# awaelchli/torch-optical-flow

Hardware: AMD Instinct MI355X
Metric: image-pairs/sec + corr-lookup HBM GB/s, RAFT 12-iter @ Sintel 1024×436 (higher is better)
Workload: dtype corr + convs split-fp16 (22-bit operands: fp16 hi + lo, 3 f16 MFMA per product, fp32 accumulate); lookup fp32; 1 GPU; raft-12iter-sintel-436x1024; pairs_per_gpu=8, global_batch=8, iters=12, padded=440x1024, parallelism=pairs sharded over 1 GPU(s), conv_benchmark=True, update_impl=split, hip_graph=True, steps_in_flight=1, full=False

## Files before the change

### include/oflow.h

```cpp
#ifndef OFLOW_H_
#define OFLOW_H_

#ifdef __cplusplus
extern "C" {
#endif

#define OFLOW_ABI_VERSION 1

#define OFLOW_OK 0
#define OFLOW_E_NULL (-1)
#define OFLOW_E_SHAPE (-2)
#define OFLOW_E_LEVELS (-3)
#define OFLOW_E_TINY (-4)
#define OFLOW_E_RADIUS (-5)
#define OFLOW_E_MODE (-6)
#define OFLOW_E_ALIGN (-7)

#define OFLOW_MAX_LEVELS 8
#define OFLOW_MAX_RADIUS 7

#define OFLOW_INTERP_BILINEAR 0
#define OFLOW_INTERP_NEAREST 1
#define OFLOW_INTERP_BICUBIC 2
#define OFLOW_PAD_ZEROS 0
#define OFLOW_PAD_BORDER 1
#define OFLOW_PAD_REFLECTION 2

#define OFLOW_IN_S32 0
#define OFLOW_IN_F32_NORM 1
#define OFLOW_IN_F32 2
#define OFLOW_IN_IMG7S2 3
#define OFLOW_IN_FLOW7 4
#define OFLOW_EPI_FLOW_HEAD 3

int oflow_abi_version(void);
const char* oflow_status_string(int status);

int oflow_corr_pyramid_dims(int H, int W, int num_levels, int* level_h, int* level_w);

int oflow_corr_pyramid_f32(const float* d_fmap1, const float* d_fmap2, int B, int C, int H, int W,
                           int num_levels, float* const* d_levels, void* stream);

int oflow_corr_lookup_f32(const float* const* d_levels, const int* level_h, const int* level_w,
                          int num_levels, const float* d_coords, int B, int H, int W, int radius,
                          float* d_out, void* stream);

long long oflow_corr_tiled_level_floats(int H_l, int W_l);
int oflow_corr_pyramid_tiled_f32(const float* d_fmap1, const float* d_fmap2, int B, int C, int H, int W,
                                 int num_levels, float* const* d_levels, void* stream);
int oflow_corr_pyramid_tiled_s32(const void* d_fmap1_s32, const void* d_fmap2_s32, int B, int C, int H, int W,
                                 int num_levels, float* const* d_levels, void* stream);
int oflow_corr_lookup_tiled_f32(const float* const* d_levels, const int* level_h, const int* level_w,
                                int num_levels, const float* d_coords, int B, int H, int W, int radius,
                                float* d_out, void* stream);
int oflow_corr_untile_f32(const float* d_tiled, float* d_out, long long Q, int H_l, int W_l, void* stream);

int oflow_grid_warp_f32(const float* d_frame, const float* d_flow, int B, int C, int H, int W, int mode,
                        int padding_mode, int align_corners, float* d_out, void* stream);

int oflow_grid_sample_f32(const float* d_input, const float* d_grid, int B, int C, int H, int W, int Ho, int Wo,
                          int mode, int padding_mode, int align_corners, float* d_out, void* stream);

int oflow_corr_otf_prepare_f16(const float* d_fmap1, const float* d_fmap2, int B, int C, int H, int W,
                               int num_levels, void* d_f1h, void* const* d_f2h, float* d_scratch, void* stream);
int oflow_corr_lookup_otf_f16(const void* d_f1h, const void* const* d_f2h, const int* level_h, const int* level_w,
                              int num_levels, const float* d_coords, int B, int C, int H, int W, int radius,
                              float* d_out, void* stream);

int oflow_bias_act_f32(const float* d_x, long long sx, const float* d_bias, float* d_y0, long long sy0, float* d_y1,
                       long long sy1, int B, int C, int P, int activation, float scale, void* stream);
int oflow_gru_reset_f32(const float* d_zr, long long szr, const float* d_br, const float* d_h, long long sh,
                        float* d_rh, long long srh, int B, int CH, int P, void* stream);
int oflow_gru_blend_f32(const float* d_zr, long long szr, const float* d_bz, const float* d_q, long long sq,
                        const float* d_bq, float* d_h, long long sh, int B, int CH, int P, void* stream);

int oflow_conv_s32(const void* d_x, long long x_pixel_stride, int in_groups, const void* d_wpack, int n_pad,
                   const float* d_wscale, const float* d_bias, int N, int B, int H, int W, int kh, int kw, int block_n,
                   int epilogue, int activation, float out_scale, void* d_y0, long long y0_pixel_stride, void* d_y1,
                   long long y1_pixel_stride, float* d_f32, long long f32_batch_stride, long long f32_channel_stride,
                   int f32_accumulate, float* d_gru_h, float* d_gru_z, int gru_channels, void* stream);
int oflow_pack_s32_f32(const float* d_x, long long x_batch_stride, int C, int B, int H, int W, int activation,
                       int dst_channel, void* d_y0, long long y0_pixel_stride, void* d_y1, long long y1_pixel_stride,
                       float* d_nhwc, int nhwc_pixel_stride, void* stream);
int oflow_flow_prep_s32(const float* d_coords, int B, int H, int W, void* d_patches, void* d_flow0,
                        long long flow0_pixel_stride, void* d_flow1, long long flow1_pixel_stride, void* stream);
int oflow_flow_head_col2im_f32(const float* d_y, const float* d_bias, int B, int H, int W, float* d_coords, void* stream);
int oflow_flow_head_finish_f32(const float* d_partial, int slabs, const float* d_bias, int B, int H, int W,
                               float* d_coords, void* d_flow0, long long flow0_pixel_stride, void* d_flow1,
                               long long flow1_pixel_stride, void* stream);

int oflow_normalize_images_f32(const float* d_x0, const float* d_x1, long long n, float* d_y0, float* d_y1, void* stream);

int oflow_replicate_pad_f32(const float* const* d_src, float* const* d_dst, int count, long long planes, int H, int W,
                            int top, int bottom, int left, int right, void* stream);

int oflow_set_range_flag(unsigned int* d_flag);

int oflow_range_flag_exchange(unsigned int* d_flag, unsigned int* d_out, void* stream);

int oflow_timing_event_create(void** ev);
int oflow_timing_event_destroy(void* ev);
int oflow_timing_event_record(void* ev, void* stream, int external);
int oflow_timing_event_elapsed_ms(void* start, void* end, float* ms);

int oflow_flow_head2_s32(const void* d_x, long long x_pixel_stride, int in_groups, const float* d_weight,
                         const float* d_bias, int B, int H, int W, float* d_coords, void* stream);
int oflow_flow_head2_tiled_s32(const void* d_x, long long x_pixel_stride, int in_groups, const float* d_wr,
                               const float* d_bias, int B, int H, int W, float* d_coords, void* stream);
int oflow_corr_lookup_tiled_nhwc_f32(const float* const* d_levels, const int* level_h, const int* level_w, int num_levels,
                                     const float* d_coords, int B, int H, int W, int radius, float* d_out, int row_floats,
                                     void* stream);
int oflow_corr_lookup_convc1_s32(const float* const* d_levels, const int* level_h, const int* level_w, int num_levels,
                                 const float* d_coords, int B, int H, int W, int radius, const void* d_wpack,
                                 const float* d_wscale, const float* d_bias, void* d_y, long long y_pixel_stride,
                                 void* stream);

int oflow_conv_s32_ex(const void* d_x, long long x_pixel_stride, int in_groups, const void* d_wpack, int n_pad,
                      const float* d_wscale, const float* d_bias, int N, int B, int H, int W, int kh, int kw,
                      int block_n, int epilogue, int activation, float out_scale, void* d_y0, long long y0_pixel_stride,
                      void* d_y1, long long y1_pixel_stride, float* d_f32, long long f32_batch_stride,
                      long long f32_channel_stride, int f32_accumulate, float* d_gru_h, float* d_gru_z,
                      int gru_channels, float* d_nhwc, int nhwc_pixel_stride, float* d_stats, const void* d_res,
                      long long res_pixel_stride, int res_activation, int s2d, void* stream);
int oflow_conv_s32_ex2(const void* d_x, long long x_pixel_stride, int in_groups, const void* d_wpack, int n_pad,
                       const float* d_wscale, const float* d_bias, int N, int B, int H, int W, int kh, int kw,
                       int block_n, int epilogue, int activation, float out_scale, void* d_y0, long long y0_pixel_stride,
                       void* d_y1, long long y1_pixel_stride, float* d_f32, long long f32_batch_stride,
                       long long f32_channel_stride, int f32_accumulate, float* d_gru_h, float* d_gru_z,
                       int gru_channels, float* d_nhwc, int nhwc_pixel_stride, float* d_stats, const void* d_res,
                       long long res_pixel_stride, int res_activation, int s2d, int in_format,
                       const float* d_in_scale, const float* d_in_shift, void* stream);
int oflow_conv_s32_ex3(const void* d_x, long long x_pixel_stride, int in_groups, const void* d_wpack, int n_pad,
                       const float* d_wscale, const float* d_bias, int N, int B, int H, int W, int kh, int kw,
                       int block_n, int epilogue, int activation, float out_scale, void* d_y0, long long y0_pixel_stride,
                       void* d_y1, long long y1_pixel_stride, float* d_f32, long long f32_batch_stride,
                       long long f32_channel_stride, int f32_accumulate, float* d_gru_h, float* d_gru_z,
                       int gru_channels, float* d_nhwc, int nhwc_pixel_stride, float* d_stats, const void* d_res,
                       long long res_pixel_stride, int res_activation, int s2d, int in_format,
                       const float* d_in_scale, const float* d_in_shift, const float* d_addend,
                       long long addend_pixel_stride, void* stream);
int oflow_conv_s32_ex4(const void* d_x, long long x_pixel_stride, int in_groups, const void* d_wpack, int n_pad,
                       const float* d_wscale, const float* d_bias, int N, int B, int H, int W, int kh, int kw,
                       int block_n, int epilogue, int activation, float out_scale, void* d_y0, long long y0_pixel_stride,
                       void* d_y1, long long y1_pixel_stride, float* d_f32, long long f32_batch_stride,
                       long long f32_channel_stride, int f32_accumulate, float* d_gru_h, float* d_gru_z,
                       int gru_channels, float* d_nhwc, int nhwc_pixel_stride, float* d_stats, const void* d_res,
                       long long res_pixel_stride, int res_activation, int s2d, int in_format,
                       const float* d_in_scale, const float* d_in_shift, const float* d_addend,
                       long long addend_pixel_stride, const void* d_wfrag, void* stream);
int oflow_conv_s32_ex5(const void* d_x, long long x_pixel_stride, int in_groups, const void* d_wpack, int n_pad,
                       const float* d_wscale, const float* d_bias, int N, int B, int H, int W, int kh, int kw,
                       int block_n, int epilogue, int activation, float out_scale, void* d_y0, long long y0_pixel_stride,
                       void* d_y1, long long y1_pixel_stride, float* d_f32, long long f32_batch_stride,
                       long long f32_channel_stride, int f32_accumulate, float* d_gru_h, float* d_gru_z,
                       int gru_channels, float* d_nhwc, int nhwc_pixel_stride, float* d_stats, const void* d_res,
                       long long res_pixel_stride, int res_activation, int s2d, int in_format,
                       const float* d_in_scale, const float* d_in_shift, const float* d_addend,
                       long long addend_pixel_stride, const void* d_wfrag, float* d_ksplit_slab,
                       unsigned* d_ksplit_ctr, long long ksplit_tiles, void* stream);
int oflow_conv_s32_ex6(const void* d_x, long long x_pixel_stride, int in_groups, const void* d_wpack, int n_pad,
                       const float* d_wscale, const float* d_bias, int N, int B, int H, int W, int kh, int kw,
                       int block_n, int epilogue, int activation, float out_scale, void* d_y0, long long y0_pixel_stride,
                       void* d_y1, long long y1_pixel_stride, float* d_f32, long long f32_batch_stride,
                       long long f32_channel_stride, int f32_accumulate, float* d_gru_h, float* d_gru_z,
                       int gru_channels, float* d_nhwc, int nhwc_pixel_stride, float* d_stats, const void* d_res,
                       long long res_pixel_stride, int res_activation, int s2d, int in_format,
                       const float* d_in_scale, const float* d_in_shift, const float* d_addend,
                       long long addend_pixel_stride, const void* d_wfrag, float* d_ksplit_slab,
                       unsigned* d_ksplit_ctr, long long ksplit_tiles, const float* d_fh_weights, float* d_fh_partial,
                       int fh_slabs, void* stream);
int oflow_stem_patches_s32(const float* d_img, int B, int C, int H, int W, void* d_out, int out_groups, void* stream);
int oflow_norm_stats_finalize(const float* d_partials, int B, int tiles, int n_pad, int C, double eps, float* d_alpha,
                              float* d_beta, void* stream);
int oflow_norm_apply_s32(const float* d_x, int C, int B, int H, int W, const float* d_alpha, const float* d_beta,
                         int activation, int res_mode, const void* d_res, long long res_pixel_stride, const float* d_x2,
                         const float* d_alpha2, const float* d_beta2, int res_activation, int s2d, void* d_y,
                         long long y_pixel_stride, void* stream);

int oflow_convex_upsample_f32(const float* d_flow, const float* d_mask, int B, int H, int W, float* d_out, void* stream);

int oflow_corr_lookup_backward_f32(const float* d_grad_out, const float* d_coords, int B, int H, int W, int radius,
                                   float* const* d_grad_levels, const int* level_h, const int* level_w, int num_levels,
                                   void* stream);
int oflow_corr_pyramid_grad_combine_f32(float* const* d_grad_levels, const int* level_h, const int* level_w,
                                        int num_levels, long long Q, void* stream);
int oflow_corr_fmap_grad_f32(const float* d_fmap1, const float* d_fmap2, const float* d_g0, int B, int C, int N,
                             float scale, float* d_grad_f1, float* d_grad_f2, void* stream);

int oflow_grid_warp_backward_f32(const float* d_grad_out, const float* d_frame, const float* d_flow, int B, int C, int H,
                                 int W, int mode, int padding_mode, int align_corners, float* d_grad_frame,
                                 float* d_grad_flow, void* stream);
int oflow_grid_sample_backward_f32(const float* d_grad_out, const float* d_input, const float* d_grid, int B, int C,
                                   int H, int W, int Ho, int Wo, int mode, int padding_mode, int align_corners,
                                   float* d_grad_input, float* d_grad_grid, void* stream);

#define OFLOW_FLOW_STATS_CHUNKS 128
#define OFLOW_FLOW2RGB_BAKER 0
#define OFLOW_FLOW2RGB_HSV 1
#define OFLOW_FLOW2RGB_MEISTER 2
int oflow_flow_stats_f32(const float* d_flow, int B, int H, int W, int clip, float clip_lo, float clip_hi,
                         int invert_y, float* d_partials, void* stream);
int oflow_flow2rgb_f32(const float* d_flow, int B, int H, int W, int method, int clip, float clip_lo, float clip_hi,
                       int invert_y, int have_denom, float denom, const float* d_partials, float* d_rgb, void* stream);
int oflow_flow_pack_f32(const float* d_flow, int B, int H, int W, int channels, int flip_rows, float* d_out,
                        void* stream);

#define OFLOW_FLOW_METRICS_PARTIALS 1024
#define OFLOW_MAX_PREDS 32
#define OFLOW_VALID_NONE 0
#define OFLOW_VALID_F32 1
#define OFLOW_VALID_U8 2
int oflow_flow_error_stats_f32(const float* d_pred, long long pred_sb, long long pred_sc, long long pred_sh,
                               const float* d_target, long long target_sb, long long target_sc, long long target_sh,
                               const void* d_valid, int valid_kind, long long valid_sb, long long valid_sh, int B, int H,
                               int W, float abs_threshold, float rel_threshold, float max_flow, float* d_epe_map,
                               double* d_workspace, double* d_accum, void* stream);
int oflow_sequence_loss_f32(const float* const* d_preds, int n_preds, const float* weights, const float* d_flow_gt,
                            const void* d_valid, int valid_kind, int B, int H, int W, float max_flow,
                            double* d_workspace, float* d_loss, double* d_stats, void* stream);
int oflow_sequence_loss_backward_f32(const float* d_grad_out, const float* const* d_preds, float* const* d_grads,
                                     int n_preds, const float* weights, const float* d_flow_gt, const void* d_valid,
                                     int valid_kind, int B, int H, int W, float max_flow, void* stream);

#ifdef __cplusplus
}
#endif

#endif
```

### torch-optical-flow_amd/csrc/conv_s32.hip

```cpp
#include "oflow_internal.h"

namespace oflow {
namespace {

typedef _Float16 half8 __attribute__((ext_vector_type(8)));
typedef float f32x16 __attribute__((ext_vector_type(16)));
typedef unsigned int u32x4 __attribute__((ext_vector_type(4)));

__device__ __forceinline__ int swz(int row) { return (row >> 1) & 7; }
#ifndef OFLOW_BREG_RING
#define OFLOW_BREG_RING 2
#endif
#ifndef OFLOW_VSLIDE
#define OFLOW_VSLIDE 1
#endif
#ifndef OFLOW_XCD_MAP
#define OFLOW_XCD_MAP 0
#endif
#ifndef OFLOW_STEM_SINGLE_A
#define OFLOW_STEM_SINGLE_A 1
#endif
#ifndef OFLOW_PAD_ROWS
#define OFLOW_PAD_ROWS 1
#endif
#ifndef OFLOW_HALO_DB
#define OFLOW_HALO_DB 0
#endif

constexpr int kTY = 4, kTX = 32;

#ifdef OFLOW_ABLATE
#define OFLOW_ABL(bit) ((a.exp_flags & (bit)) != 0)
#else
#define OFLOW_ABL(bit) false
#endif
constexpr int kAinGroups = 4;


struct ConvArgs {
  const uint8_t* x;
  long long xps;
  int kg;
  const uint8_t* w;
  int npad;
  const float* wsc;
  const float* bias;
  int N;
  int B, H, W, tiles_x, tiles_y;
  int act;
  float oscale;
  uint8_t* y0;
  long long y0ps;
  uint8_t* y1;
  long long y1ps;
  float* f;
  long long fbs, fcs;
  int faccum;
  float* h;
  float* z;
  int gch;
  const float* add;
  long long addps;
  float* fn;
  int fnps;
  float* stats;
  const uint8_t* res;
  long long resps;
  int res_act;
  int s2d;
  const float* ia;
  const float* ib;
  int ain;
  int cin;
  int wbytes;
  const uint8_t* wf;
  int exp_flags;
  float* ks_slab;
  unsigned* ks_ctr;
  long long ks_tiles;
  const float* fhw;
  float* fhy;
};
constexpr int kEpiFlowHead = OFLOW_EPI_FLOW_HEAD;
constexpr int kInS32 = OFLOW_IN_S32, kInF32Norm = OFLOW_IN_F32_NORM, kInF32 = OFLOW_IN_F32, kInImg = OFLOW_IN_IMG7S2,
              kInFlow = OFLOW_IN_FLOW7;
constexpr int kImgC = 3, kImgK = 7, kImgRows = (kTY - 1) * 2 + kImgK, kImgCols = (kTX - 1) * 2 + kImgK;
constexpr int kImgHalf = (kImgCols + 1) / 2, kImgPitch = 2 * kImgHalf, kImgPlane = kImgRows * kImgPitch;

__device__ __forceinline__ float sigmoid_hw(float v) {
  return __builtin_amdgcn_rcpf(1.0f + __builtin_amdgcn_exp2f(v * -1.4426950408889634f));
}
__device__ __forceinline__ float tanh_hw(float v) {
  return 1.0f - 2.0f * __builtin_amdgcn_rcpf(__builtin_amdgcn_exp2f(v * 2.8853900817779268f) + 1.0f);
}

__device__ __forceinline__ float act_fn(float v, int act) {
  if (act == 1) return v < 0.f ? 0.f : v;
  if (act == 2) return 1.0f / (1.0f + expf(-v));
  if (act == 3) return tanhf(v);
  return v;
}

__device__ __forceinline__ void split8(const float* v, half8& hi, half8& lo) { split_vec(v, hi, lo); }

__device__ __forceinline__ void store_s32(uint8_t* y, long long ps, long long P, int n, int N, const float* v, float& gm) {
  uint8_t* line = y + P * ps + (long long)(n >> 5) * 128 + ((n & 31) >> 3) * 16;
  if (n + 8 <= N) {
    half8 hi, lo;
    split8(v, hi, lo);
    gm = fmaxf(gm, fmaxf(fmaxf(fmaxf(fabsf(v[0]), fabsf(v[1])), fmaxf(fabsf(v[2]), fabsf(v[3]))),
                         fmaxf(fmaxf(fabsf(v[4]), fabsf(v[5])), fmaxf(fabsf(v[6]), fabsf(v[7])))));
    *reinterpret_cast<half8*>(line) = hi;
    *reinterpret_cast<half8*>(line + 64) = lo;
  } else {
    _Float16* hp = reinterpret_cast<_Float16*>(line);
    _Float16* lp = reinterpret_cast<_Float16*>(line + 64);
#pragma unroll
    for (int j = 0; j < 8; ++j) {
      if (n + j < N) {
        gm = fmaxf(gm, fabsf(v[j]));
        _Float16 h_, l_;
        split_f16(v[j], h_, l_);
        hp[j] = h_;
        lp[j] = l_;
      }
    }
  }
}

typedef __attribute__((address_space(4))) const float cfloat;
template <int T0, int T1>
__device__ __forceinline__ void flow_head_partials(const float* tp, cfloat* w, float* yp, long long plane, bool in) {
  constexpr int NO = 2 * (T1 - T0);
  float acc[2][NO];
#pragma unroll
  for (int j = 0; j < NO; ++j) acc[0][j] = acc[1][j] = 0.f;
  float wn[2][NO];
#pragma unroll
  for (int e = 0; e < 2; ++e)
#pragma unroll
    for (int j = 0; j < NO; ++j) wn[e][j] = w[e * 18 + 2 * T0 + j];
  float2 tn = *reinterpret_cast<const float2*>(tp);
#pragma unroll
  for (int e = 0; e < 2; ++e)
#pragma unroll
    for (int j = 0; j < NO; ++j) asm volatile("" : "+s"(wn[e][j]));
  asm volatile("" : "+v"(tn.x), "+v"(tn.y));
#pragma unroll 2
  for (int c0 = 0; c0 < 64; c0 += 2) {
    float wc[2][NO];
#pragma unroll
    for (int e = 0; e < 2; ++e)
#pragma unroll
      for (int j = 0; j < NO; ++j) wc[e][j] = wn[e][j];
    const float2 t = tn;
    const int c1 = c0 + 2 < 64 ? c0 + 2 : c0;
#pragma unroll
    for (int e = 0; e < 2; ++e)
#pragma unroll
      for (int j = 0; j < NO; ++j) wn[e][j] = w[(c1 + e) * 18 + 2 * T0 + j];
    tn = *reinterpret_cast<const float2*>(tp + c1);
    __builtin_amdgcn_sched_barrier(0);
#pragma unroll
    for (int j = 0; j < NO; ++j) {
      acc[0][j] = fmaf(t.x, wc[0][j], acc[0][j]);
      acc[1][j] = fmaf(t.y, wc[1][j], acc[1][j]);
    }
    __builtin_amdgcn_sched_barrier(0);
#pragma unroll
    for (int e = 0; e < 2; ++e)
#pragma unroll
      for (int j = 0; j < NO; ++j) asm volatile("" : "+s"(wn[e][j]));
    asm volatile("" : "+v"(tn.x), "+v"(tn.y));
  }
  if (in) {
#pragma unroll
    for (int j = 0; j < NO; ++j) yp[(2 * T0 + j) * plane] = acc[0][j] + acc[1][j];
  }
}

template <int KH, int KW, int BN, int WM, int WN, int EPI, int TY = kTY, int AIN = kInS32, bool BREG = false, int BD = 1>
__global__ __launch_bounds__(64 * WM * WN, WM * WN == 8 ? 1 : 2) void conv_s32_kernel(ConvArgs a) {
  constexpr int NTH = 64 * WM * WN;
  constexpr int T = KH * KW;
  constexpr int BM = TY * kTX;
  constexpr int PH = KH / 2, PW = KW / 2;
  constexpr int HY = TY + KH - 1, HX = kTX + KW - 1, NPIX = HY * HX;
  constexpr int AITEMS = NPIX * 8, APER = (AITEMS + NTH - 1) / NTH;
  constexpr int BITEMS = BN * 8, BPER = (BITEMS + NTH - 1) / NTH;
  constexpr int MT = TY / WM;
  constexpr int NT = BN / WN / 32;
  static_assert((WM * WN == 4 || WM * WN == 8) && MT >= 1 && NT >= 1, "bad wave grid");
  static_assert(NTH % 8 == 0, "an A item's 16-B chunk is tid & 7");
  constexpr bool WIN = AIN == kInImg || AIN == kInFlow;
  constexpr int WC = AIN == kInFlow ? 2 : kImgC, WS = AIN == kInFlow ? 1 : 2;
  constexpr int WROWS = (kTY - 1) * WS + kImgK, WCOLS = (kTX - 1) * WS + kImgK;
  constexpr int WHALF = WS == 2 ? (WCOLS + 1) / 2 : WCOLS, WPITCH = WS == 2 ? 2 * WHALF : WCOLS;
  constexpr int WPLANE = WROWS * WPITCH;
  constexpr int WKPAD = AIN == kInFlow ? 128 : 160;
  constexpr int WAPER = WIN ? BM * 4 / NTH : 1;
  static_assert(!WIN || (BM * 4) % NTH == 0, "window items");
  static_assert(AIN != kInImg || (WHALF == kImgHalf && WPITCH == kImgPitch && WPLANE == kImgPlane), "stem window");
  constexpr bool ADB = (T == 1) && !(WIN && OFLOW_STEM_SINGLE_A);
  constexpr int RS = 128;
  constexpr int RSA = (BREG || OFLOW_PAD_ROWS) ? 144 : RS, RSB = OFLOW_PAD_ROWS ? 144 : RS;
  constexpr int A_BYTES = NPIX * RSA, B_BYTES = BN * RSB;
  static_assert(!BREG || (T > 1 && (WM == 1 || WM == 2 || WM == 4) && BN == 32 * WN && AIN == kInS32),
                "register-direct B: T > 1, WM x WN waves of one 32-channel tile each");
  constexpr bool HDB = BREG && OFLOW_HALO_DB;
  constexpr int MAIN_BYTES = ((ADB || HDB) ? 2 : 1) * A_BYTES + (BREG ? 0 : 2 * B_BYTES);
  constexpr int TS = BN + 4;
  constexpr int EPI_BYTES = BM * TS * 4;
  constexpr int LDS_BYTES = MAIN_BYTES > EPI_BYTES ? MAIN_BYTES : EPI_BYTES;
  constexpr int kImgZero = WC * WPLANE;
  constexpr int IMG_FLOATS = (kImgZero + 1 + 3) & ~3;
  constexpr int AFF_BYTES = AIN == kInF32Norm ? kAinGroups * 32 * 8
                            : WIN ? IMG_FLOATS * 4 + WKPAD * 4
                            : 0;
  static_assert(!WIN || (T == 1 && TY == kTY), "window input: 1x1 geometry over the patch channels, 4-row tiles");
  __shared__ __attribute__((aligned(16))) uint8_t smem[LDS_BYTES + AFF_BYTES];
  __shared__ float2 sSB[BN];
  __shared__ float3 sStat[EPI == 0 ? WM * BN : 1];
  float2* sAff = reinterpret_cast<float2*>(smem + LDS_BYTES);
  float* sImg = reinterpret_cast<float*>(smem + LDS_BYTES);
  int* sKoff = reinterpret_cast<int*>(smem + LDS_BYTES + (WIN ? IMG_FLOATS * 4 : 0));
  uint8_t* sA = smem;
  uint8_t* sB = smem + (ADB ? 2 : 1) * A_BYTES;

  const int tid = threadIdx.x, lane = tid & 63, wave = tid >> 6;
  const int wm = wave / WN, wn = wave % WN;
  const int r = lane & 31, hh = lane >> 5;
  if constexpr (BREG) {
    if (a.ks_slab != nullptr) {
      const int z = blockIdx.z;
      a.x += (long long)z * a.kg * 128;
      a.wf += (long long)z * a.kg * T * a.npad * 128;
    }
  }
  auto aswz = [](int p) { return (BREG || OFLOW_PAD_ROWS) ? 0 : swz(p); };
  auto bswz = [](int n) { return OFLOW_PAD_ROWS ? 0 : swz(n); };

  int tile, cblk;
  if constexpr (OFLOW_XCD_MAP) {
    const int nblk = a.npad / BN, ntiles = a.tiles_x * a.tiles_y * a.B, bid = blockIdx.x;
    const int full = (ntiles >> 3) * 8 * nblk;
    if (bid < full) {
      const int grp = bid / (8 * nblk), rem = bid - grp * 8 * nblk;
      cblk = rem >> 3;
      tile = grp * 8 + (rem & 7);
    } else {
      const int ntail = ntiles & 7, rem = bid - full;
      cblk = rem / ntail;
      tile = (ntiles & ~7) + (rem - cblk * ntail);
    }
  } else {
    tile = blockIdx.x;
    cblk = blockIdx.y;
  }
  const int tx0 = (tile % a.tiles_x) * kTX;
  tile /= a.tiles_x;
  const int ty0 = (tile % a.tiles_y) * TY;
  const int b = tile / a.tiles_y;
  const int n0 = cblk * BN;
  const long long pix0 = (long long)b * a.H * a.W;

  u32x4 ra[APER], rb[BPER];
  const __amdgpu_buffer_rsrc_t rsA = __builtin_amdgcn_make_buffer_rsrc(
      const_cast<uint8_t*>(a.x + pix0 * a.xps), (short)0, (int)((long long)a.H * a.W * a.xps), 0x00020000);
  const __amdgpu_buffer_rsrc_t rsB =
      __builtin_amdgcn_make_buffer_rsrc(const_cast<uint8_t*>(a.w), (short)0, a.wbytes, 0x00020000);
  auto a_off = [&](int s_, int& col) {
    int t_ = tid;
    asm volatile("" : "+v"(t_));
    const int item = (AITEMS % NTH == 0) ? t_ + s_ * NTH : min(t_ + s_ * NTH, AITEMS - 1);
    const int p = item >> 3, c = item & 7;
    const int gy = ty0 - PH + p / HX, gx = tx0 - PW + p % HX;
    const int cy = min(max(gy, 0), a.H - 1), cx = min(max(gx, 0), a.W - 1);
    col = c * 16;
    return (cy * a.W + cx) * (int)a.xps + (AIN == kInF32 ? 0 : c * 16);
  };
  unsigned aok = 0u;
#pragma unroll
  for (int s_ = 0; s_ < APER; ++s_) {
    const int item = (AITEMS % NTH == 0) ? tid + s_ * NTH : min(tid + s_ * NTH, AITEMS - 1);
    const int p = item >> 3;
    const int gy = ty0 - PH + p / HX, gx = tx0 - PW + p % HX;
    const bool ok = static_cast<unsigned>(gy) < static_cast<unsigned>(a.H) && static_cast<unsigned>(gx) < static_cast<unsigned>(a.W);
    aok |= (ok ? 1u : 0u) << s_;
  }
  int boff[BPER];
#pragma unroll
  for (int s_ = 0; s_ < BPER; ++s_) boff[s_] = (n0 + (tid + s_ * NTH) / 8) * 128 + ((tid + s_ * NTH) & 7) * 16;
#define OFLOW_LOAD_A(RA, G)                                                                                          \
  if constexpr (!WIN) _Pragma("unroll") for (int s_ = 0; s_ < APER; ++s_) {                                        \
    int col_;                                                                                                        \
    const int off_ = a_off(s_, col_);                                                                                \
    if constexpr (AIN == kInF32)    \
      RA[s_] = __builtin_amdgcn_raw_buffer_load_b128(rsA, off_ + min((G) * 128 + col_, a.cin * 4 - 16), 0, 0);      \
    else                                                                                                             \
      RA[s_] = __builtin_amdgcn_raw_buffer_load_b128(rsA, off_, (G) * 128, 0);                                      \
  }
#define OFLOW_WRITE_A(RA, BUF, G)                                                                                    \
  if (!OFLOW_ABL(4)) {                                                                                               \
  float amx_ = 0.f;                                                                                                  \
  float2 af4_[4];                                                                                                    \
  if constexpr (AIN == kInF32Norm) _Pragma("unroll") for (int e_ = 0; e_ < 4; ++e_)                                  \
    af4_[e_] = sAff[(G) * 32 + 4 * (tid & 7) + e_];                                                                  \
  if constexpr (WIN) {                                                                                               \
                                                                                                        \
    _Pragma("unroll") for (int s_ = 0; s_ < WAPER; ++s_) {                                                           \
      const int item = tid + s_ * NTH;                                                                               \
      const int p = item % BM, cp = item / BM;                                                                       \
      const int pb_ = WS * (p >> 5) * WPITCH + (p & 31);                                                             \
      const int4 k0_ = *reinterpret_cast<const int4*>(sKoff + (G) * 32 + 8 * cp);                                    \
      const int4 k1_ = *reinterpret_cast<const int4*>(sKoff + (G) * 32 + 8 * cp + 4);                                \
      const int kov_[8] = {k0_.x, k0_.y, k0_.z, k0_.w, k1_.x, k1_.y, k1_.z, k1_.w};                                  \
      float v8_[8];                                                                                                  \
      _Pragma("unroll") for (int e_ = 0; e_ < 8; ++e_) {                                                             \
        v8_[e_] = sImg[kov_[e_] < 0 ? kImgZero : pb_ + kov_[e_]];                                                    \
        amx_ = fmaxf(amx_, fabsf(v8_[e_]));                                                                          \
      }                                                                                                              \
      half8 h8_, l8_;                                                                                                \
      split_vec(v8_, h8_, l8_);                                                                                      \
      uint8_t* rw_ = sA + (BUF) * A_BYTES + p * RSA;                                                                 \
      *reinterpret_cast<half8*>(rw_ + ((cp ^ aswz(p)) << 4)) = h8_;                                                  \
      *reinterpret_cast<half8*>(rw_ + (((4 + cp) ^ aswz(p)) << 4)) = l8_;                                            \
    }                                                                                                                \
  } else                                                                                                             \
  _Pragma("unroll") for (int s_ = 0; s_ < APER; ++s_) {                                                              \
    const int item = tid + s_ * NTH;                                                                            \
                                                     \
    const int p = item >> 3, c = item & 7;                                                                           \
    if (AITEMS % NTH == 0 || item < AITEMS) {                                                                   \
      if constexpr (AIN != kInS32) {                                                                                 \
                   \
        typedef _Float16 half4_ __attribute__((ext_vector_type(4)));                                                 \
        half4_ h4 = {0, 0, 0, 0}, l4 = {0, 0, 0, 0};                                                                 \
        if (((aok >> s_) & 1u) && (AIN != kInF32 || (G) * 32 + 4 * c < a.cin)) {                                     \
          const float* fv = reinterpret_cast<const float*>(&RA[s_]);                                                 \
          float mx_ = 0.f, v4_[4];                                                                                   \
          _Pragma("unroll") for (int e_ = 0; e_ < 4; ++e_) {                                                         \
            float v_ = fv[e_];                                                                                       \
            if constexpr (AIN == kInF32Norm) {                                                                       \
              const float2 af = af4_[e_];                                                                            \
              v_ = v_ * af.x + af.y;                                                                                 \
              v_ = v_ < 0.f ? 0.f : v_;                                                                              \
            }                                                                                                        \
            mx_ = fmaxf(mx_, fabsf(v_));                                                                             \
            v4_[e_] = v_;                                                                                            \
          }                                                                                                          \
          split_vec(v4_, h4, l4);                                                                                    \
          amx_ = fmaxf(amx_, mx_);                                                                                   \
        }                                                                                                            \
        uint8_t* rw_ = sA + (BUF) * A_BYTES + p * RSA + (c & 1) * 8;                                                 \
        *reinterpret_cast<half4_*>(rw_ + (((c >> 1) ^ aswz(p)) << 4)) = h4;                                          \
        *reinterpret_cast<half4_*>(rw_ + (((4 + (c >> 1)) ^ aswz(p)) << 4)) = l4;                                    \
      } else {                                                                                                       \
        *reinterpret_cast<u32x4*>(sA + (BUF) * A_BYTES + p * RSA + ((c ^ aswz(p)) << 4)) =                          \
            ((aok >> s_) & 1u) ? RA[s_] : u32x4{0u, 0u, 0u, 0u};                                                     \
      }                                                                                                              \
    }                                                                                                                \
  }                                                                                                                  \
  if constexpr (AIN != kInS32) range_guard(amx_);                                                                    \
  }
#define OFLOW_LOAD_B(RB, STEP)                                                                                       \
  _Pragma("unroll") for (int s_ = 0; s_ < BPER; ++s_) {                                                              \
    const int item = tid + s_ * NTH;                                                                            \
    if (BITEMS % NTH == 0 || item < BITEMS)                                                                     \
      RB[s_] = __builtin_amdgcn_raw_buffer_load_b128(rsB, boff[s_], (STEP) * a.npad * 128, 0);                      \
  }
#define OFLOW_WRITE_B(RB, BUF)                                                                                       \
  if (!OFLOW_ABL(32)) _Pragma("unroll") for (int s_ = 0; s_ < BPER; ++s_) {                                          \
    const int item = tid + s_ * NTH;                                                                            \
    const int n = item >> 3, c = item & 7;                                                                           \
    if (BITEMS % NTH == 0 || item < BITEMS)                                                                     \
      *reinterpret_cast<u32x4*>(sB + (BUF) * B_BYTES + n * RSB + ((c ^ bswz(n)) << 4)) = RB[s_];                    \
  }
#define OFLOW_READ_OPS(AH, AL, BH, BL, I, S_)                                                                        \
  {                                                                                                                  \
    const int ii_ = (I);                                                                                              \
    const int t_ = ii_ % T, ky_ = t_ / KW, kx_ = t_ - ky_ * KW;                                                       \
    const uint8_t* bufA_ = sA + (ADB ? (ii_ & 1) * A_BYTES : 0);                                                      \
    const uint8_t* bufB_ = sB + (ii_ & 1) * B_BYTES;                                                                  \
    const int chi_ = 2 * (S_) + hh, clo_ = 4 + 2 * (S_) + hh;                                                        \
    _Pragma("unroll") for (int mt_ = 0; mt_ < MT; ++mt_) {                                                           \
      const int p_ = (wm * MT + mt_ + ky_) * HX + r + kx_;                                                           \
      const uint8_t* row_ = bufA_ + p_ * RSA;                                                                        \
      AH[mt_] = *reinterpret_cast<const half8*>(row_ + ((chi_ ^ aswz(p_)) << 4));                                    \
      AL[mt_] = *reinterpret_cast<const half8*>(row_ + ((clo_ ^ aswz(p_)) << 4));                                    \
    }                                                                                                                \
    _Pragma("unroll") for (int nt_ = 0; nt_ < NT; ++nt_) {                                                           \
      const int n_ = wn * (BN / WN) + nt_ * 32 + r;                                                                  \
      const uint8_t* row_ = bufB_ + n_ * RSB;                                                                        \
      BH[nt_] = *reinterpret_cast<const half8*>(row_ + ((chi_ ^ bswz(n_)) << 4));                                    \
      BL[nt_] = *reinterpret_cast<const half8*>(row_ + ((clo_ ^ bswz(n_)) << 4));                                    \
    }                                                                                                                \
  }
#define OFLOW_MFMAS(AH, AL, BH, BL)                                                                                  \
  if (!OFLOW_ABL(2)) _Pragma("unroll") for (int mt = 0; mt < MT; ++mt)                                               \
    _Pragma("unroll") for (int nt = 0; nt < NT; ++nt) {                                                              \
      acc[mt][nt] = __builtin_amdgcn_mfma_f32_32x32x16_f16(AH[mt], BL[nt], acc[mt][nt], 0, 0, 0);                    \
      acc[mt][nt] = __builtin_amdgcn_mfma_f32_32x32x16_f16(AL[mt], BH[nt], acc[mt][nt], 0, 0, 0);                    \
      acc[mt][nt] = __builtin_amdgcn_mfma_f32_32x32x16_f16(AH[mt], BH[nt], acc[mt][nt], 0, 0, 0);                    \
    }

  f32x16 acc[MT][NT];
#pragma unroll
  for (int i = 0; i < MT; ++i)
#pragma unroll
    for (int j = 0; j < NT; ++j)
#pragma unroll
      for (int e = 0; e < 16; ++e) acc[i][j][e] = 0.f;

  const int S = a.kg * T;
  for (int c = tid; c < BN; c += NTH) {
    const int n = min(n0 + c, a.N - 1);
    sSB[c] = make_float2(a.wsc[n], a.bias ? a.bias[n] : 0.f);
  }
  if constexpr (AIN == kInF32Norm) {
    for (int e = tid; e < a.kg * 32; e += NTH)
      sAff[e] = make_float2(a.ia[(long long)b * a.kg * 32 + e], a.ib[(long long)b * a.kg * 32 + e]);
    __syncthreads();
  }
  if constexpr (AIN == kInImg) {
    const float* img = reinterpret_cast<const float*>(a.x) + (long long)b * kImgC * (2 * a.H) * (2 * a.W);
    const int iy0 = 2 * ty0 - kImgK / 2, ix0 = 2 * tx0 - kImgK / 2;
    constexpr int IMG_N = kImgC * kImgRows * kImgCols, IMG_PER = (IMG_N + NTH - 1) / NTH;
    if (a.exp_flags & 1) {
      for (int e = tid; e < IMG_N; e += NTH) {
        const int ch = e / (kImgRows * kImgCols), rem = e - ch * (kImgRows * kImgCols);
        const int ry = rem / kImgCols, rx = rem - ry * kImgCols;
        const int iy = iy0 + ry, ix = ix0 + rx;
        float v = 0.f;
        if (static_cast<unsigned>(iy) < static_cast<unsigned>(2 * a.H) && static_cast<unsigned>(ix) < static_cast<unsigned>(2 * a.W))
          v = img[((long long)ch * (2 * a.H) + iy) * (2 * a.W) + ix];
        sImg[ch * kImgPlane + ry * kImgPitch + (rx & 1) * kImgHalf + (rx >> 1)] = v;
      }
    } else {
    float iv[IMG_PER];
    int io[IMG_PER];
#pragma unroll
    for (int s_ = 0; s_ < IMG_PER; ++s_) {
      const int e = min(tid + s_ * NTH, IMG_N - 1);
      const int ch = e / (kImgRows * kImgCols), rem = e - ch * (kImgRows * kImgCols);
      const int ry = rem / kImgCols, rx = rem - ry * kImgCols;
      const int iy = iy0 + ry, ix = ix0 + rx;
      const bool in = static_cast<unsigned>(iy) < static_cast<unsigned>(2 * a.H) && static_cast<unsigned>(ix) < static_cast<unsigned>(2 * a.W);
      const int cy = min(max(iy, 0), 2 * a.H - 1), cx = min(max(ix, 0), 2 * a.W - 1);
      const float v = img[((long long)ch * (2 * a.H) + cy) * (2 * a.W) + cx];
      iv[s_] = in ? v : 0.f;
      io[s_] = ch * kImgPlane + ry * kImgPitch + (rx & 1) * kImgHalf + (rx >> 1);
    }
#pragma unroll
    for (int s_ = 0; s_ < IMG_PER; ++s_)
      if (tid + s_ * NTH < IMG_N) sImg[io[s_]] = iv[s_];
    }
  }
  if constexpr (AIN == kInFlow) {
    const float* co = reinterpret_cast<const float*>(a.x) + (long long)b * 2 * a.H * a.W;
    const int iy0 = ty0 - kImgK / 2, ix0 = tx0 - kImgK / 2;
    constexpr int FL_N = 2 * WROWS * WCOLS, FL_PER = (FL_N + NTH - 1) / NTH;
    float iv[FL_PER];
    int io[FL_PER];
#pragma unroll
    for (int s_ = 0; s_ < FL_PER; ++s_) {
      const int e = min(tid + s_ * NTH, FL_N - 1);
      const int ch = e / (WROWS * WCOLS), rem = e - ch * (WROWS * WCOLS);
      const int ry = rem / WCOLS, rx = rem - ry * WCOLS;
      const int iy = iy0 + ry, ix = ix0 + rx;
      const bool in = static_cast<unsigned>(iy) < static_cast<unsigned>(a.H) && static_cast<unsigned>(ix) < static_cast<unsigned>(a.W);
      const int cy = min(max(iy, 0), a.H - 1), cx = min(max(ix, 0), a.W - 1);
      const float v = co[((long long)ch * a.H + cy) * a.W + cx] - static_cast<float>(ch == 0 ? ix : iy);
      iv[s_] = in ? v : 0.f;
      io[s_] = ch * WPLANE + ry * WPITCH + rx;
    }
#pragma unroll
    for (int s_ = 0; s_ < FL_PER; ++s_)
      if (tid + s_ * NTH < FL_N) sImg[io[s_]] = iv[s_];
  }
  if constexpr (WIN) {
    for (int k = tid; k < WKPAD; k += NTH) {
      const int t = k / WC, ch = k - t * WC;
      const int ky = t / kImgK, kx = t - ky * kImgK;
      sKoff[k] = t < kImgK * kImgK
                     ? ch * WPLANE + ky * WPITCH + (WS == 2 ? (kx & 1) * WHALF + (kx >> 1) : kx)
                     : -1;
    }
    if (tid == 0) sImg[kImgZero] = 0.f;
    __syncthreads();
  }
  if constexpr (BREG) {
  const __amdgpu_buffer_rsrc_t rsW =
      __builtin_amdgcn_make_buffer_rsrc(const_cast<uint8_t*>(a.wf), (short)0, a.wbytes, 0x00020000);
  const int wlane = ((n0 >> 5) + wn) * 4096 + lane * 16;
  const int wstep = a.npad * 128;
  constexpr int RING = (T == 5 && KH == 5 && EPI == 0) ? 2 : OFLOW_BREG_RING;
  u32x4 bq[RING][4];
  auto load_b = [&](u32x4 (&d)[4], int step) {
#pragma unroll
    for (int e = 0; e < 4; ++e) d[e] = __builtin_amdgcn_raw_buffer_load_b128(rsW, wlane + e * 1024, step * wstep, 0);
  };
#define OFLOW_READ_A(AH, AL, I, S_)                                                                                   \
  {                                                                                                                  \
    const int ii_ = (I);                                                                                              \
    const int t_ = ii_ % T, ky_ = t_ / KW, kx_ = t_ - ky_ * KW;                                                       \
    const int chi_ = 2 * (S_) + hh, clo_ = 4 + 2 * (S_) + hh;                                                        \
    const uint8_t* sAb_ = sA + (HDB && ((ii_ / T) & 1) ? A_BYTES : 0);           \
    _Pragma("unroll") for (int mt_ = 0; mt_ < MT; ++mt_) {                                                           \
      const int p_ = (wm * MT + mt_ + ky_) * HX + r + kx_;                                                           \
      const uint8_t* row_ = sAb_ + p_ * RSA;                                                                         \
      AH[mt_] = *reinterpret_cast<const half8*>(row_ + (chi_ << 4));                                                 \
      AL[mt_] = *reinterpret_cast<const half8*>(row_ + (clo_ << 4));                                                 \
    }                                                                                                                \
  }
#define OFLOW_MFMAS_R(AH, AL, BC, S_)                                                                                 \
  if (!OFLOW_ABL(2)) _Pragma("unroll") for (int mt = 0; mt < MT; ++mt) {                                             \
    const half8 bh_ = __builtin_bit_cast(half8, BC[2 * (S_)]), bl_ = __builtin_bit_cast(half8, BC[2 * (S_) + 1]);     \
    acc[mt][0] = __builtin_amdgcn_mfma_f32_32x32x16_f16(AH[mt], bl_, acc[mt][0], 0, 0, 0);                           \
    acc[mt][0] = __builtin_amdgcn_mfma_f32_32x32x16_f16(AL[mt], bh_, acc[mt][0], 0, 0, 0);                           \
    acc[mt][0] = __builtin_amdgcn_mfma_f32_32x32x16_f16(AH[mt], bh_, acc[mt][0], 0, 0, 0);                           \
  }
#pragma unroll
  for (int q = 0; q < RING; ++q) load_b(bq[q], q < S ? q : S - 1);
  OFLOW_LOAD_A(ra, 0);
  OFLOW_WRITE_A(ra, 0, 0);
  OFLOW_LOAD_A(ra, a.kg > 1 ? 1 : 0);
  __syncthreads();
  constexpr int GPB = (T % RING == 0) ? 1 : RING;
  constexpr bool VSLIDE = OFLOW_VSLIDE && KW == 1 && KH > 1 && WM == 1 && !(EPI == 0 && KH == 5);
  if constexpr (VSLIDE) {
    constexpr int NR = MT + KH - 1;
    half8 V[NR][2][2];
    auto rd = [&](int hr, int sub, int grp) {
      const uint8_t* row_ = sA + (HDB && (grp & 1) ? A_BYTES : 0) + (hr * HX + r) * RSA;
      V[hr][sub][0] = *reinterpret_cast<const half8*>(row_ + ((2 * sub + hh) << 4));
      V[hr][sub][1] = *reinterpret_cast<const half8*>(row_ + ((4 + 2 * sub + hh) << 4));
    };
    auto mf = [&](int ky, int sub, u32x4 (&bc)[4]) {
      if (OFLOW_ABL(2)) return;
      const half8 bh_ = __builtin_bit_cast(half8, bc[2 * sub]), bl_ = __builtin_bit_cast(half8, bc[2 * sub + 1]);
#pragma unroll
      for (int mt = 0; mt < MT; ++mt) {
        acc[mt][0] = __builtin_amdgcn_mfma_f32_32x32x16_f16(V[mt + ky][sub][0], bl_, acc[mt][0], 0, 0, 0);
        acc[mt][0] = __builtin_amdgcn_mfma_f32_32x32x16_f16(V[mt + ky][sub][1], bh_, acc[mt][0], 0, 0, 0);
        acc[mt][0] = __builtin_amdgcn_mfma_f32_32x32x16_f16(V[mt + ky][sub][0], bh_, acc[mt][0], 0, 0, 0);
      }
    };
#pragma unroll
    for (int m = 0; m < MT; ++m) rd(m, 0, 0);
    for (int g0 = 0; g0 < a.kg; g0 += GPB) {
#pragma unroll
      for (int j = 0; j < GPB * T; ++j) {
        const int gg = g0 + j / T, t = j % T;
        if (GPB > 1 && j > 0 && t == 0 && gg >= a.kg) break;
        const int i_ = gg * T + t;
        u32x4 (&bc)[4] = bq[j % RING];
        if (t == 0) {
#pragma unroll
          for (int m = 0; m < MT; ++m) rd(m, 1, gg);
        } else {
          rd(t + MT - 1, 1, gg);
        }
        mf(t, 0, bc);
        if (t == T - 1) {
          if constexpr (HDB) {
            OFLOW_WRITE_A(ra, (gg + 1) & 1, gg + 1 < a.kg ? gg + 1 : gg);
          } else {
            __syncthreads();
            OFLOW_WRITE_A(ra, 0, gg + 1 < a.kg ? gg + 1 : gg);
          }
          const int g2 = gg + 2 < a.kg ? gg + 2 : a.kg - 1;
          OFLOW_LOAD_A(ra, g2);
          __syncthreads();
#pragma unroll
          for (int m = 0; m < MT; ++m) rd(m, 0, gg + 1);
        } else {
          rd(t + MT, 0, gg);
        }
        mf(t, 1, bc);
        load_b(bc, i_ + RING < S ? i_ + RING : S - 1);
      }
    }
  } else {
  half8 xah[MT], xal[MT], yah[MT], yal[MT];
  OFLOW_READ_A(xah, xal, 0, 0);
  for (int g0 = 0; g0 < a.kg; g0 += GPB) {
#pragma unroll
    for (int j = 0; j < GPB * T; ++j) {
      const int gg = g0 + j / T, t = j % T;
      if (GPB > 1 && j > 0 && t == 0 && gg >= a.kg) break;
      const int i_ = gg * T + t;
      u32x4 (&bc)[4] = bq[j % RING];
      OFLOW_READ_A(yah, yal, i_, 1);
      OFLOW_MFMAS_R(xah, xal, bc, 0);
      if (t == T - 1) {
        if constexpr (HDB) {
          OFLOW_WRITE_A(ra, (gg + 1) & 1, gg + 1 < a.kg ? gg + 1 : gg);
        } else {
          __syncthreads();
          OFLOW_WRITE_A(ra, 0, gg + 1 < a.kg ? gg + 1 : gg);
        }
        const int g2 = gg + 2 < a.kg ? gg + 2 : a.kg - 1;
        OFLOW_LOAD_A(ra, g2);
        __syncthreads();
      }
      OFLOW_READ_A(xah, xal, i_ + 1, 0);
      OFLOW_MFMAS_R(yah, yal, bc, 1);
      load_b(bc, i_ + RING < S ? i_ + RING : S - 1);
    }
  }
  }
#undef OFLOW_READ_A
#undef OFLOW_MFMAS_R
  } else {
  u32x4 rbr[BD][BPER];
  u32x4 rar[ADB ? BD : 1][APER];
  OFLOW_LOAD_B(rbr[0], 0);
  OFLOW_LOAD_A(rar[0], 0);
  OFLOW_WRITE_A(rar[0], 0, 0);
  OFLOW_WRITE_B(rbr[0], 0);
#pragma unroll
  for (int d = 1; d <= BD; ++d) {
    const int id = d < S ? d : S - 1;
    OFLOW_LOAD_B(rbr[d % BD], id);
    if constexpr (ADB) { OFLOW_LOAD_A(rar[d % BD], id); }
  }
  if constexpr (!ADB) { OFLOW_LOAD_A(rar[0], a.kg > 1 ? 1 : 0); }
  __syncthreads();
  half8 xah[MT], xal[MT], xbh[NT], xbl[NT];
  half8 yah[MT], yal[MT], ybh[NT], ybl[NT];
  OFLOW_READ_OPS(xah, xal, xbh, xbl, 0, 0);

  constexpr int GPB2 = (BD > 1 && (T % BD) != 0) ? BD : 1;
  for (int g0 = 0; g0 < a.kg; g0 += GPB2) {
#pragma unroll
    for (int j = 0; j < GPB2 * T; ++j) {
      const int g = g0 + j / T, t = j % T;
      if (GPB2 > 1 && j > 0 && t == 0 && g >= a.kg) break;
      const int i_ = g * T + t;
      u32x4 (&rb)[BPER] = rbr[(j + 1) % BD];
      OFLOW_WRITE_B(rb, (i_ + 1) & 1);
      if constexpr (ADB) { OFLOW_WRITE_A(rar[(j + 1) % BD], (i_ + 1) & 1, i_ + 1 < S ? i_ + 1 : S - 1); }
      {
        const int i2 = i_ + 1 + BD < S ? i_ + 1 + BD : S - 1;
        OFLOW_LOAD_B(rb, i2);
        if constexpr (ADB) { OFLOW_LOAD_A(rar[(j + 1) % BD], i2); }
      }
      OFLOW_READ_OPS(yah, yal, ybh, ybl, i_, 1);
      OFLOW_MFMAS(xah, xal, xbh, xbl);
      if constexpr (!ADB) {
        if (t == T - 1) {
          __syncthreads();
          OFLOW_WRITE_A(rar[0], 0, g + 1 < a.kg ? g + 1 : g);
          const int g2 = g + 2 < a.kg ? g + 2 : a.kg - 1;
          OFLOW_LOAD_A(rar[0], g2);
        }
      }
      if (!OFLOW_ABL(64)) __syncthreads();
      OFLOW_READ_OPS(xah, xal, xbh, xbl, i_ + 1, 0);
      OFLOW_MFMAS(yah, yal, ybh, ybl);
    }
  }
  }
#undef OFLOW_MFMAS
#undef OFLOW_READ_OPS
#undef OFLOW_LOAD_A
#undef OFLOW_WRITE_A
#undef OFLOW_LOAD_B
#undef OFLOW_WRITE_B

  if constexpr (BREG) {
    if (a.ks_slab != nullptr) {
      typedef __attribute__((address_space(1))) unsigned gu32;
      __shared__ unsigned sTicket;
      const int tile_id = blockIdx.y * gridDim.x + blockIdx.x;
      gu32* ctr = (gu32*)(a.ks_ctr) + 2 * tile_id;
      if (tid == 0) sTicket = __hip_atomic_fetch_add(ctr, 1u, __ATOMIC_RELAXED, __HIP_MEMORY_SCOPE_AGENT);
      __syncthreads();
      const unsigned ticket = sTicket;
      const __amdgpu_buffer_rsrc_t rsS = __builtin_amdgcn_make_buffer_rsrc(
          a.ks_slab + (size_t)tile_id * (BM * BN), (short)0, BM * BN * 4, 0x00020000);
      const int sbase = wave * (MT * NT * 4096) + lane * 16;
      if ((ticket & 1u) == 0u) {
#pragma unroll
        for (int mt = 0; mt < MT; ++mt)
#pragma unroll
          for (int nt = 0; nt < NT; ++nt)
#pragma unroll
            for (int e4 = 0; e4 < 4; ++e4) {
              const u32x4 v = {__float_as_uint(acc[mt][nt][4 * e4]), __float_as_uint(acc[mt][nt][4 * e4 + 1]),
                               __float_as_uint(acc[mt][nt][4 * e4 + 2]), __float_as_uint(acc[mt][nt][4 * e4 + 3])};
              __builtin_amdgcn_raw_buffer_store_b128(v, rsS, sbase + ((mt * NT + nt) * 4 + e4) * 1024, 0, 16);
            }
        asm volatile("s_waitcnt vmcnt(0)" ::: "memory");
        __syncthreads();
        if (tid == 0) __hip_atomic_fetch_add(ctr + 1, 1u, __ATOMIC_RELAXED, __HIP_MEMORY_SCOPE_AGENT);
        return;
      }
      if (tid == 0) {
        const unsigned want = (ticket >> 1) + 1u;
        for (unsigned spin = 0; spin < (1u << 24); ++spin) {
          if (static_cast<int>(__hip_atomic_load(ctr + 1, __ATOMIC_RELAXED, __HIP_MEMORY_SCOPE_AGENT) - want) >= 0) break;
          __builtin_amdgcn_s_sleep(1);
        }
        __builtin_amdgcn_fence(__ATOMIC_ACQUIRE, "agent");
        asm volatile("s_waitcnt vmcnt(0)" ::: "memory");
      }
      __syncthreads();
#pragma unroll
      for (int mt = 0; mt < MT; ++mt)
#pragma unroll
        for (int nt = 0; nt < NT; ++nt) {
          u32x4 pv[4];
#pragma unroll
          for (int e4 = 0; e4 < 4; ++e4)
            pv[e4] = __builtin_amdgcn_raw_buffer_load_b128(rsS, sbase + ((mt * NT + nt) * 4 + e4) * 1024, 0, 0);
#pragma unroll
          for (int e4 = 0; e4 < 4; ++e4)
#pragma unroll
            for (int j = 0; j < 4; ++j) acc[mt][nt][4 * e4 + j] += __uint_as_float(pv[e4][j]);
        }
    }
  }

  constexpr int C8 = BN / 8;
  constexpr int KIT = (BM * C8 + NTH - 1) / NTH;
  constexpr bool GRU = EPI == 1 || EPI == 2;
  const bool has_add = GRU && a.add != nullptr;
  u32x4 ad[GRU ? KIT : 1][2];
  if (has_add) {
#pragma unroll
    for (int k = 0; k < (GRU ? KIT : 0); ++k) {
      const int item = tid + k * NTH;
      const int pl = item / C8, n = n0 + (item - pl * C8) * 8;
      const int y = ty0 + pl / kTX, x = tx0 + (pl % kTX);
      if (item >= BM * C8 || n >= a.N || y >= a.H || x >= a.W) continue;
      const u32x4* ap = reinterpret_cast<const u32x4*>(a.add + (pix0 + (long long)y * a.W + x) * a.addps + n);
      ad[k][0] = ap[0];
      ad[k][1] = ap[1];
    }
  }
  __syncthreads();
  float* sT = reinterpret_cast<float*>(smem);
#pragma unroll
  for (int mt = 0; mt < MT; ++mt)
#pragma unroll
    for (int nt = 0; nt < NT; ++nt) {
      const int nl = wn * (BN / WN) + nt * 32 + r;
      const int pbase = (wm * MT + mt) * kTX;
      if constexpr (EPI == kEpiFlowHead) {
        const float2 sb = sSB[nl];
#pragma unroll
        for (int e = 0; e < 16; ++e) {
          const int m = (e & 3) + 8 * (e >> 2) + 4 * hh;
          const float v = fmaf(acc[mt][nt][e], sb.x, sb.y);
          sT[(pbase + m) * TS + nl] = v < 0.f ? 0.f : v;
        }
      } else {
#pragma unroll
      for (int e = 0; e < 16; ++e) {
        const int m = (e & 3) + 8 * (e >> 2) + 4 * hh;
        sT[(pbase + m) * TS + nl] = acc[mt][nt][e];
      }
      }
    }
  if constexpr (EPI == 0 && TY >= kTY) {
    if (a.stats != nullptr && !OFLOW_ABL(8)) {
#pragma unroll
      for (int nt = 0; nt < NT; ++nt) {
        const int nl = wn * (BN / WN) + nt * 32 + r;
        const float2 sb = sSB[nl];
        float cnt = 0.f, sum = 0.f, q = 0.f;
        const bool full = ty0 + TY <= a.H && tx0 + kTX <= a.W;
        if (full) {
#pragma unroll
          for (int mt = 0; mt < MT; ++mt)
#pragma unroll
            for (int e = 0; e < 16; ++e) sum += acc[mt][nt][e] * sb.x + sb.y;
          cnt = 16.f * MT;
        } else {
#pragma unroll
          for (int mt = 0; mt < MT; ++mt) {
            const bool yok = ty0 + wm * MT + mt < a.H;
#pragma unroll
            for (int e = 0; e < 16; ++e) {
              const bool ok = yok && tx0 + (e & 3) + 8 * (e >> 2) + 4 * hh < a.W;
              sum += ok ? acc[mt][nt][e] * sb.x + sb.y : 0.f;
              cnt += ok ? 1.f : 0.f;
            }
          }
        }
        const float mean = cnt > 0.f ? sum / cnt : 0.f;
        if (full) {
#pragma unroll
          for (int mt = 0; mt < MT; ++mt)
#pragma unroll
            for (int e = 0; e < 16; ++e) {
              const float d = (acc[mt][nt][e] * sb.x + sb.y) - mean;
              float dd = d * d;
              asm volatile("" : "+v"(dd));
              q += dd;
            }
        } else {
#pragma unroll
          for (int mt = 0; mt < MT; ++mt) {
            const bool yok = ty0 + wm * MT + mt < a.H;
#pragma unroll
            for (int e = 0; e < 16; ++e) {
              const bool ok = yok && tx0 + (e & 3) + 8 * (e >> 2) + 4 * hh < a.W;
              const float d = (acc[mt][nt][e] * sb.x + sb.y) - mean;
              q += ok ? d * d : 0.f;
            }
          }
        }
        const float nb = __shfl_xor(cnt, 32), mb = __shfl_xor(mean, 32), qb = __shfl_xor(q, 32);
        const float n0_ = hh ? nb : cnt, m0_ = hh ? mb : mean, q0_ = hh ? qb : q;
        const float n1_ = hh ? cnt : nb, m1_ = hh ? mean : mb, q1_ = hh ? q : qb;
        const float nn = n0_ + n1_;
// ... 445 lines not shown

using namespace oflow;

extern "C" int oflow_conv_s32_ex5(const void* d_x, long long x_pixel_stride, int in_groups, const void* d_wpack,
                                  int n_pad, const float* d_wscale, const float* d_bias, int N, int B, int H, int W, int kh,
                                  int kw, int block_n, int epilogue, int activation, float out_scale, void* d_y0,
                                  long long y0_pixel_stride, void* d_y1, long long y1_pixel_stride, float* d_f32,
                                  long long f32_batch_stride, long long f32_channel_stride, int f32_accumulate,
                                  float* d_gru_h, float* d_gru_z, int gru_channels, float* d_nhwc, int nhwc_pixel_stride,
                                  float* d_stats, const void* d_res, long long res_pixel_stride, int res_activation,
                                  int s2d, int in_format, const float* d_in_scale, const float* d_in_shift,
                                  const float* d_addend, long long addend_pixel_stride, const void* d_wfrag,
                                  float* d_ksplit_slab, unsigned* d_ksplit_ctr, long long ksplit_tiles, void* stream);

extern "C" int oflow_conv_s32_ex4(const void* d_x, long long x_pixel_stride, int in_groups, const void* d_wpack,
                                  int n_pad, const float* d_wscale, const float* d_bias, int N, int B, int H, int W, int kh,
                                  int kw, int block_n, int epilogue, int activation, float out_scale, void* d_y0,
                                  long long y0_pixel_stride, void* d_y1, long long y1_pixel_stride, float* d_f32,
                                  long long f32_batch_stride, long long f32_channel_stride, int f32_accumulate,
                                  float* d_gru_h, float* d_gru_z, int gru_channels, float* d_nhwc, int nhwc_pixel_stride,
                                  float* d_stats, const void* d_res, long long res_pixel_stride, int res_activation,
                                  int s2d, int in_format, const float* d_in_scale, const float* d_in_shift,
                                  const float* d_addend, long long addend_pixel_stride, const void* d_wfrag, void* stream) {
  return oflow_conv_s32_ex5(d_x, x_pixel_stride, in_groups, d_wpack, n_pad, d_wscale, d_bias, N, B, H, W, kh, kw,
                            block_n, epilogue, activation, out_scale, d_y0, y0_pixel_stride, d_y1, y1_pixel_stride,
                            d_f32, f32_batch_stride, f32_channel_stride, f32_accumulate, d_gru_h, d_gru_z, gru_channels,
                            d_nhwc, nhwc_pixel_stride, d_stats, d_res, res_pixel_stride, res_activation, s2d, in_format,
                            d_in_scale, d_in_shift, d_addend, addend_pixel_stride, d_wfrag, nullptr, nullptr, 0, stream);
}

extern "C" int oflow_conv_s32_ex5(const void* d_x, long long x_pixel_stride, int in_groups, const void* d_wpack,
                                  int n_pad, const float* d_wscale, const float* d_bias, int N, int B, int H, int W, int kh,
                                  int kw, int block_n, int epilogue, int activation, float out_scale, void* d_y0,
                                  long long y0_pixel_stride, void* d_y1, long long y1_pixel_stride, float* d_f32,
                                  long long f32_batch_stride, long long f32_channel_stride, int f32_accumulate,
                                  float* d_gru_h, float* d_gru_z, int gru_channels, float* d_nhwc, int nhwc_pixel_stride,
                                  float* d_stats, const void* d_res, long long res_pixel_stride, int res_activation,
                                  int s2d, int in_format, const float* d_in_scale, const float* d_in_shift,
                                  const float* d_addend, long long addend_pixel_stride, const void* d_wfrag,
                                  float* d_ksplit_slab, unsigned* d_ksplit_ctr, long long ksplit_tiles, void* stream) {
  ConvArgs a;
  const int st = build_conv_args(a, d_x, x_pixel_stride, in_groups, d_wpack, n_pad, d_wscale, d_bias, N, B, H, W, kh, kw,
                                 block_n, epilogue, activation, out_scale, d_y0, y0_pixel_stride, d_y1, y1_pixel_stride,
                                 d_f32, f32_batch_stride, f32_channel_stride, f32_accumulate, d_gru_h, d_gru_z,
                                 gru_channels, d_nhwc, nhwc_pixel_stride, d_stats, d_res, res_pixel_stride,
                                 res_activation, s2d);
  if (st != OFLOW_OK) return st;
  if (d_wfrag) {
    if ((uintptr_t)d_wfrag & 15) return OFLOW_E_ALIGN;
    if (n_pad % 32) return OFLOW_E_SHAPE;
    a.wf = static_cast<const uint8_t*>(d_wfrag);
  }
  if (in_format < kInS32 || in_format > kInFlow) return OFLOW_E_MODE;
  if (in_format == kInFlow) {
    if (kh != 1 || kw != 1 || epilogue != 0 || block_n != 128 || in_groups != (kImgK * kImgK * 2 + 31) / 32)
      return OFLOW_E_MODE;
    if ((long long)2 * B * H * W >= (1ll << 31) || d_addend) return OFLOW_E_SHAPE;
    a.ain = in_format;
    return dispatch_conv(a, kh, kw, block_n, epilogue, static_cast<hipStream_t>(stream));
  }
  if (in_format == kInImg) {
    if (kh != 1 || kw != 1 || epilogue != 0 || block_n != 64 || in_groups != (kImgK * kImgK * kImgC + 31) / 32)
      return OFLOW_E_MODE;
    if ((long long)kImgC * 4 * H * W >= (1ll << 31)) return OFLOW_E_SHAPE;
    a.ain = in_format;
    if (d_addend) return OFLOW_E_MODE;
    return dispatch_conv(a, kh, kw, block_n, epilogue, static_cast<hipStream_t>(stream));
  }
  if (in_format != kInF32 && (x_pixel_stride & 127)) return OFLOW_E_ALIGN;
  if (in_format == kInF32Norm && x_pixel_stride != (long long)in_groups * 128) return OFLOW_E_SHAPE;
  if (in_format == kInF32) {
    const long long cin = x_pixel_stride / 4;
    if ((x_pixel_stride & 15) || cin > (long long)in_groups * 32 || cin <= (long long)(in_groups - 1) * 32) return OFLOW_E_SHAPE;
    a.cin = static_cast<int>(cin);
  }
  if (in_format == kInF32Norm) {
    if (!d_in_scale || !d_in_shift) return OFLOW_E_NULL;
    if (kh != 3 || kw != 3 || epilogue != 0 || in_groups > kAinGroups) return OFLOW_E_MODE;
    a.ia = d_in_scale;
    a.ib = d_in_shift;
  } else if (in_format == kInF32) {
    if (kh != 1 || kw != 1 || epilogue != 0 || block_n != 128) return OFLOW_E_MODE;
  }
  a.ain = in_format;
  if (d_addend) {
    if (epilogue == 0) return OFLOW_E_MODE;
    if (N % 8) return OFLOW_E_SHAPE;
    if (((uintptr_t)d_addend & 15) || (addend_pixel_stride & 3) || addend_pixel_stride < N) return OFLOW_E_ALIGN;
    a.add = d_addend;
    a.addps = addend_pixel_stride;
  }
  if (d_ksplit_slab || d_ksplit_ctr) {
    if (!d_ksplit_slab || !d_ksplit_ctr) return OFLOW_E_NULL;
    if (((uintptr_t)d_ksplit_slab & 15) || ((uintptr_t)d_ksplit_ctr & 7)) return OFLOW_E_ALIGN;
    if (ksplit_tiles <= 0) return OFLOW_E_SHAPE;
    a.ks_slab = d_ksplit_slab;
    const bool breg = in_format == kInS32 && a.wf != nullptr && use_breg(a, block_n, kh * kw) && kh * kw != 4 &&
                      (block_n == 128 || (kh == 3 && kw == 3)) && (epilogue == 0 || kh * kw == 5);
    a.ks_slab = nullptr;
    if (breg && (in_groups % 2) == 0) {
      if ((long long)B * ((H + kTY - 1) / kTY) * ((W + kTX - 1) / kTX) * (n_pad / block_n) > ksplit_tiles)
        return OFLOW_E_SHAPE;
      a.ks_slab = d_ksplit_slab;
      a.ks_ctr = d_ksplit_ctr;
      a.ks_tiles = ksplit_tiles;
      a.kg = in_groups / 2;
      a.wbytes /= 2;
    }
  }
  return dispatch_conv(a, kh, kw, block_n, epilogue, static_cast<hipStream_t>(stream));
}

extern "C" int oflow_conv_s32_ex6(const void* d_x, long long x_pixel_stride, int in_groups, const void* d_wpack,
                                  int n_pad, const float* d_wscale, const float* d_bias, int N, int B, int H, int W, int kh,
                                  int kw, int block_n, int epilogue, int activation, float out_scale, void* d_y0,
                                  long long y0_pixel_stride, void* d_y1, long long y1_pixel_stride, float* d_f32,
                                  long long f32_batch_stride, long long f32_channel_stride, int f32_accumulate,
                                  float* d_gru_h, float* d_gru_z, int gru_channels, float* d_nhwc, int nhwc_pixel_stride,
                                  float* d_stats, const void* d_res, long long res_pixel_stride, int res_activation,
                                  int s2d, int in_format, const float* d_in_scale, const float* d_in_shift,
                                  const float* d_addend, long long addend_pixel_stride, const void* d_wfrag,
                                  float* d_ksplit_slab, unsigned* d_ksplit_ctr, long long ksplit_tiles,
                                  const float* d_fh_weights, float* d_fh_partial, int fh_slabs, void* stream) {
  if (epilogue != kEpiFlowHead)
    return oflow_conv_s32_ex5(d_x, x_pixel_stride, in_groups, d_wpack, n_pad, d_wscale, d_bias, N, B, H, W, kh, kw,
                              block_n, epilogue, activation, out_scale, d_y0, y0_pixel_stride, d_y1, y1_pixel_stride,
                              d_f32, f32_batch_stride, f32_channel_stride, f32_accumulate, d_gru_h, d_gru_z,
                              gru_channels, d_nhwc, nhwc_pixel_stride, d_stats, d_res, res_pixel_stride, res_activation,
                              s2d, in_format, d_in_scale, d_in_shift, d_addend, addend_pixel_stride, d_wfrag,
                              d_ksplit_slab, d_ksplit_ctr, ksplit_tiles, stream);
  if (!d_fh_weights || !d_fh_partial) return OFLOW_E_NULL;
  if (N != 256 || n_pad != 256 || fh_slabs != N / 64 || kh != 3 || kw != 3 || (block_n != 64 && block_n != 128))
    return OFLOW_E_SHAPE;
  if (in_format != kInS32 || activation != 1 || out_scale != 1.0f || d_y0 || d_y1 || d_f32 || d_gru_h || d_gru_z ||
      d_nhwc || d_stats || d_res || s2d || d_addend || d_ksplit_slab || d_ksplit_ctr)
    return OFLOW_E_MODE;
  if ((x_pixel_stride & 127) || ((uintptr_t)d_fh_weights & 3) || ((uintptr_t)d_fh_partial & 3)) return OFLOW_E_ALIGN;
  ConvArgs a;
  const int st = build_conv_args(a, d_x, x_pixel_stride, in_groups, d_wpack, n_pad, d_wscale, d_bias, N, B, H, W, kh, kw,
                                 block_n, 0, activation, out_scale, nullptr, 0, nullptr, 0, d_fh_partial, 0, 0, 0, nullptr,
                                 nullptr, 0, nullptr, 0, nullptr, nullptr, 0, 0, 0);
  if (st != OFLOW_OK) return st;
  a.f = nullptr;
  a.fhw = d_fh_weights;
  a.fhy = d_fh_partial;
  if (d_wfrag) {
    if ((uintptr_t)d_wfrag & 15) return OFLOW_E_ALIGN;
    a.wf = static_cast<const uint8_t*>(d_wfrag);
  }
  a.ain = kInS32;
  return dispatch_conv(a, kh, kw, block_n, epilogue, static_cast<hipStream_t>(stream));
}

extern "C" int oflow_conv_s32_ex3(const void* d_x, long long x_pixel_stride, int in_groups, const void* d_wpack,
                                  int n_pad, const float* d_wscale, const float* d_bias, int N, int B, int H, int W, int kh,
                                  int kw, int block_n, int epilogue, int activation, float out_scale, void* d_y0,
                                  long long y0_pixel_stride, void* d_y1, long long y1_pixel_stride, float* d_f32,
                                  long long f32_batch_stride, long long f32_channel_stride, int f32_accumulate,
                                  float* d_gru_h, float* d_gru_z, int gru_channels, float* d_nhwc, int nhwc_pixel_stride,
                                  float* d_stats, const void* d_res, long long res_pixel_stride, int res_activation,
                                  int s2d, int in_format, const float* d_in_scale, const float* d_in_shift,
                                  const float* d_addend, long long addend_pixel_stride, void* stream) {
  return oflow_conv_s32_ex4(d_x, x_pixel_stride, in_groups, d_wpack, n_pad, d_wscale, d_bias, N, B, H, W, kh, kw,
                            block_n, epilogue, activation, out_scale, d_y0, y0_pixel_stride, d_y1, y1_pixel_stride,
                            d_f32, f32_batch_stride, f32_channel_stride, f32_accumulate, d_gru_h, d_gru_z, gru_channels,
                            d_nhwc, nhwc_pixel_stride, d_stats, d_res, res_pixel_stride, res_activation, s2d, in_format,
                            d_in_scale, d_in_shift, d_addend, addend_pixel_stride, nullptr, stream);
}

extern "C" int oflow_conv_s32_ex2(const void* d_x, long long x_pixel_stride, int in_groups, const void* d_wpack,
                                  int n_pad, const float* d_wscale, const float* d_bias, int N, int B, int H, int W, int kh,
                                  int kw, int block_n, int epilogue, int activation, float out_scale, void* d_y0,
                                  long long y0_pixel_stride, void* d_y1, long long y1_pixel_stride, float* d_f32,
                                  long long f32_batch_stride, long long f32_channel_stride, int f32_accumulate,
                                  float* d_gru_h, float* d_gru_z, int gru_channels, float* d_nhwc, int nhwc_pixel_stride,
                                  float* d_stats, const void* d_res, long long res_pixel_stride, int res_activation,
                                  int s2d, int in_format, const float* d_in_scale, const float* d_in_shift,
                                  void* stream) {
  return oflow_conv_s32_ex3(d_x, x_pixel_stride, in_groups, d_wpack, n_pad, d_wscale, d_bias, N, B, H, W, kh, kw,
                            block_n, epilogue, activation, out_scale, d_y0, y0_pixel_stride, d_y1, y1_pixel_stride,
                            d_f32, f32_batch_stride, f32_channel_stride, f32_accumulate, d_gru_h, d_gru_z, gru_channels,
                            d_nhwc, nhwc_pixel_stride, d_stats, d_res, res_pixel_stride, res_activation, s2d, in_format,
                            d_in_scale, d_in_shift, nullptr, 0, stream);
}

extern "C" int oflow_conv_s32_ex(const void* d_x, long long x_pixel_stride, int in_groups, const void* d_wpack,
                                 int n_pad, const float* d_wscale, const float* d_bias, int N, int B, int H, int W, int kh,
                                 int kw, int block_n, int epilogue, int activation, float out_scale, void* d_y0,
                                 long long y0_pixel_stride, void* d_y1, long long y1_pixel_stride, float* d_f32,
                                 long long f32_batch_stride, long long f32_channel_stride, int f32_accumulate,
                                 float* d_gru_h, float* d_gru_z, int gru_channels, float* d_nhwc, int nhwc_pixel_stride,
                                 float* d_stats, const void* d_res, long long res_pixel_stride, int res_activation,
                                 int s2d, void* stream) {
  return oflow_conv_s32_ex2(d_x, x_pixel_stride, in_groups, d_wpack, n_pad, d_wscale, d_bias, N, B, H, W, kh, kw,
                            block_n, epilogue, activation, out_scale, d_y0, y0_pixel_stride, d_y1, y1_pixel_stride,
                            d_f32, f32_batch_stride, f32_channel_stride, f32_accumulate, d_gru_h, d_gru_z, gru_channels,
                            d_nhwc, nhwc_pixel_stride, d_stats, d_res, res_pixel_stride, res_activation, s2d, kInS32,
                            nullptr, nullptr, stream);
}

extern "C" int oflow_conv_s32(const void* d_x, long long x_pixel_stride, int in_groups, const void* d_wpack, int n_pad,
                              const float* d_wscale, const float* d_bias, int N, int B, int H, int W, int kh, int kw,
                              int block_n, int epilogue, int activation, float out_scale, void* d_y0,
                              long long y0_pixel_stride, void* d_y1, long long y1_pixel_stride, float* d_f32,
                              long long f32_batch_stride, long long f32_channel_stride, int f32_accumulate,
                              float* d_gru_h, float* d_gru_z, int gru_channels, void* stream) {
  return oflow_conv_s32_ex(d_x, x_pixel_stride, in_groups, d_wpack, n_pad, d_wscale, d_bias, N, B, H, W, kh, kw,
                           block_n, epilogue, activation, out_scale, d_y0, y0_pixel_stride, d_y1, y1_pixel_stride,
                           d_f32, f32_batch_stride, f32_channel_stride, f32_accumulate, d_gru_h, d_gru_z, gru_channels,
                           nullptr, 0, nullptr, nullptr, 0, 0, 0, stream);
}

extern "C" void oflow_exp_set_small_grid_px(int pixels) { oflow::g_small_grid_px = pixels; }
extern "C" void oflow_exp_set_stats_8row(int on) { oflow::g_stats_8row = on; }
extern "C" void oflow_exp_set_conv_flags(int flags) { oflow::g_conv_exp_flags = flags; }
extern "C" void oflow_exp_set_bn64_8row(int on) { oflow::g_bn64_8row = on; }
```

### torch-optical-flow_amd/methods/raft/model/extractor.py

```python
from __future__ import annotations

import os

from typing import Optional, List, Sequence, Tuple, Union

import torch
import torch.nn as nn
from torch import Tensor

from optical_flow import _native

from .update import CONV_BLOCKS, parse_block_overrides


def _norm_layer(norm_fn: str, planes: int, groups: int) -> nn.Module:
    if norm_fn == "group":
        return nn.GroupNorm(num_groups=groups, num_channels=planes)
    if norm_fn == "batch":
        return nn.BatchNorm2d(planes)
    if norm_fn == "instance":
        return nn.InstanceNorm2d(planes)
    if norm_fn == "none":
        return nn.Sequential()
    raise ValueError(f"unknown norm_fn {norm_fn!r}")


class ResidualBlock(nn.Module):

    def __init__(self, in_planes: int, planes: int, norm_fn: str = "group", stride: int = 1) -> None:
        super().__init__()
        self.conv1 = nn.Conv2d(in_planes, planes, kernel_size=3, padding=1, stride=stride)
        self.conv2 = nn.Conv2d(planes, planes, kernel_size=3, padding=1)
        self.relu = nn.ReLU(inplace=True)
        groups = planes // 8
        self.norm1 = _norm_layer(norm_fn, planes, groups)
        self.norm2 = _norm_layer(norm_fn, planes, groups)
        if stride != 1:
            self.norm3 = _norm_layer(norm_fn, planes, groups)
            self.downsample = nn.Sequential(nn.Conv2d(in_planes, planes, kernel_size=1, stride=stride), self.norm3)
        else:
            self.downsample = None

    def forward(self, x: Tensor) -> Tensor:
        y = self.relu(self.norm1(self.conv1(x)))
        y = self.relu(self.norm2(self.conv2(y)))
        if self.downsample is not None:
            x = self.downsample(x)
        return self.relu(x + y)


class BasicEncoder(nn.Module):

    def __init__(self, output_dim: int = 128, norm_fn: str = "batch", dropout: float = 0.0) -> None:
        super().__init__()
        self.norm_fn = norm_fn
        self.norm1 = _norm_layer(norm_fn, 64, 8)
        self.conv1 = nn.Conv2d(3, 64, kernel_size=7, stride=2, padding=3)
        self.relu1 = nn.ReLU(inplace=True)
        self.in_planes = 64
        self.layer1 = self._make_layer(64, stride=1)
        self.layer2 = self._make_layer(96, stride=2)
        self.layer3 = self._make_layer(128, stride=2)
        self.conv2 = nn.Conv2d(128, output_dim, kernel_size=1)
        self.dropout = nn.Dropout2d(p=dropout) if dropout > 0 else None
        for m in self.modules():
            if isinstance(m, nn.Conv2d):
                nn.init.kaiming_normal_(m.weight, mode="fan_out", nonlinearity="relu")
            elif isinstance(m, (nn.BatchNorm2d, nn.InstanceNorm2d, nn.GroupNorm)):
                if m.weight is not None:
                    nn.init.constant_(m.weight, 1)
                if m.bias is not None:
                    nn.init.constant_(m.bias, 0)

    def _make_layer(self, dim: int, stride: int = 1) -> nn.Module:
        blocks = (ResidualBlock(self.in_planes, dim, self.norm_fn, stride=stride), ResidualBlock(dim, dim, self.norm_fn, 1))
        self.in_planes = dim
        return nn.Sequential(*blocks)

    def forward(self, x: Union[Tensor, Sequence[Tensor]]) -> Union[Tensor, Tuple[Tensor, ...]]:
        is_list = isinstance(x, (tuple, list))
        if is_list:
            batch_dim = x[0].shape[0]
            x = torch.cat(list(x), dim=0)
        x = self.relu1(self.norm1(self.conv1(x)))
        x = self.layer3(self.layer2(self.layer1(x)))
        x = self.conv2(x)
        if self.training and self.dropout is not None:
            x = self.dropout(x)
        if is_list:
            return torch.split(x, [batch_dim, batch_dim], dim=0)
        return x




def _s2d_weight(w: Tensor) -> Tensor:
    n, c = w.shape[:2]
    out = torch.zeros((n, 4, c, 2, 2), device=w.device, dtype=w.dtype)
    for kyp in range(2):
        for a in range(2):
            ky = 2 * kyp + a - 1
            if not 0 <= ky <= 2:
                continue
            for kxp in range(2):
                for b in range(2):
                    kx = 2 * kxp + b - 1
                    if 0 <= kx <= 2:
                        out[:, a * 2 + b, :, kyp, kxp] = w[:, :, ky, kx]
    return out.reshape(n, 4 * c, 2, 2)


def _fold_bn(conv: nn.Conv2d, bn: nn.Module):
    w = conv.weight.detach().double()
    b = conv.bias.detach().double() if conv.bias is not None else torch.zeros(w.shape[0], device=w.device, dtype=w.dtype)
    alpha = bn.weight.detach().double() / torch.sqrt(bn.running_var.detach().double() + bn.eps)
    beta = bn.bias.detach().double() - bn.running_mean.detach().double() * alpha
    return (w * alpha.view(-1, 1, 1, 1)).float(), (b * alpha + beta).float()


_ENC_BN_OVERRIDE = {int(k): v for k, v in
                    parse_block_overrides("OFLOW_ENC_BN", {str(b) for b in CONV_BLOCKS}).items()}


class SplitEncoder:

    def __init__(self, enc: BasicEncoder) -> None:
        if enc.norm_fn not in ("instance", "batch"):
            raise RuntimeError(f"SplitEncoder: norm_fn {enc.norm_fn!r} not supported")
        if enc.norm_fn == "batch" and enc.training:
            raise RuntimeError("SplitEncoder: batch norm needs eval mode (running statistics)")
        self.enc = enc
        self.inorm = enc.norm_fn == "instance"
        from .update import cached_pack, tensor_key

        key = tuple(tensor_key(q) for q in enc.parameters()) + tuple(tensor_key(q) for q in enc.buffers())
        self.w = cached_pack(enc, key, lambda: self._pack(enc))

    def _cw(self, conv: nn.Conv2d, norm, **kw):
        if self.inorm or norm is None:
            w, b = conv.weight, conv.bias
        else:
            w, b = _fold_bn(conv, norm)
        if kw.pop("s2d", False):
            w = _s2d_weight(w.detach().float())
        n = w.shape[0]
        return _native.ConvWeights(w, b, ((n + 31) // 32) * 32, **kw)

    def _pack(self, enc: BasicEncoder):
        W = {"stem": self._cw(enc.conv1, enc.norm1, patches=True)}
        for li, layer in enumerate((enc.layer1, enc.layer2, enc.layer3)):
            for bi, blk in enumerate(layer):
                s2 = blk.downsample is not None
                W[f"{li}.{bi}.conv1"] = self._cw(blk.conv1, blk.norm1, s2d=s2)
                W[f"{li}.{bi}.conv2"] = self._cw(blk.conv2, blk.norm2)
                if s2:
                    W[f"{li}.{bi}.down"] = self._cw(blk.downsample[0], blk.downsample[1])
        W["head"] = _native.ConvWeights(enc.conv2.weight, enc.conv2.bias, ((enc.conv2.out_channels + 31) // 32) * 32)
        return W

    @staticmethod
    def _bn(n: int) -> int:
        bn = {64: 64, 96: 96, 128: 128}.get(n, 128 if n % 128 == 0 else 64 if n % 64 == 0 else 32)
        return _ENC_BN_OVERRIDE.get(bn, bn)

    def _conv_norm(self, x, cw, shape, act, out=None, res=None, s2d=False, raw_only=False):
        b, h, w = shape
        bn = self._bn(cw.n)
        V = _native.S32Slice
        dev = x.device
        if self.inorm:
            raw = torch.empty((b * h * w, cw.n), device=dev, dtype=torch.float32)
            tiles = _native.conv_tiles(h, w)
            part = torch.empty((b, tiles, cw.n_pad, 3), device=dev, dtype=torch.float32)
            _native.conv_s32(x, cw, bn, nhwc=raw, stats=part)
            alpha, beta = _native.norm_stats(part, b, tiles, cw.n_pad, cw.n, 1e-5)
            if raw_only:
                return raw, alpha, beta
            if out is None:
                out = _native.s32_empty(b, h // 2 if s2d else h, w // 2 if s2d else w, (cw.n * (4 if s2d else 1) + 31) // 32, dev)
            if isinstance(res, _native.NhwcNormIn):
                _native.norm_apply(raw, (b, cw.n, h, w), alpha, beta, act, V(out), res_raw=(res.raw, res.scale, res.shift),
                                   res_act="relu", s2d=s2d, res_raw_relu=True)
            elif isinstance(res, tuple):
                _native.norm_apply(raw, (b, cw.n, h, w), alpha, beta, act, V(out), res_raw=res, res_act="relu", s2d=s2d)
            else:
                _native.norm_apply(raw, (b, cw.n, h, w), alpha, beta, act, V(out), res=res, res_act="relu" if res is not None else "none", s2d=s2d)
            return out
        if raw_only:
            out = _native.s32_empty(b, h, w, (cw.n + 31) // 32, dev)
            _native.conv_s32(x, cw, bn, y0=V(out))
            return out
        if out is None:
            out = _native.s32_empty(b, h // 2 if s2d else h, w // 2 if s2d else w, (cw.n * (4 if s2d else 1) + 31) // 32, dev)
        _native.conv_s32(x, cw, bn, act=act, y0=V(out), res=res, res_act="relu" if res is not None else "none", s2d=s2d)
        return out

    def _conv1(self, x, cw, shape):
        if self.inorm:
            raw, alpha, beta = self._conv_norm(x, cw, shape, "relu", raw_only=True)
            return _native.NhwcNormIn(raw, *shape, alpha, beta)
        return _native.S32Slice(self._conv_norm(x, cw, shape, "relu"))

    def stem_patches(self, x: Tensor) -> Tensor:
        x = x.float().contiguous()
        n, _, hh, ww = x.shape
        patches = _native.s32_empty(n, hh // 2, ww // 2, self.w["stem"].kg, x.device)
        _native.stem_patches(x, patches)
        return patches

    def __call__(self, x: Union[Tensor, Sequence[Tensor]], patches: Optional[Tensor] = None,
                 split_out: bool = False, stem_from_image: bool = False) -> Union[Tensor, Tuple[Tensor, ...]]:
        is_list = isinstance(x, (tuple, list))
        if is_list:
            batch_dim = x[0].shape[0]
            n, _, hh, ww = x[0].shape
            n *= len(x)
            if patches is None or tuple(patches.shape[:4]) != (n, hh // 2, ww // 2, self.w["stem"].kg):
                x = torch.cat(list(x), dim=0)
        if not isinstance(x, (tuple, list)):
            x = x.float().contiguous()
            n, _, hh, ww = x.shape
            dev = x.device
        else:
            dev = x[0].device
        if hh % 8 or ww % 8:
            raise RuntimeError("SplitEncoder: H and W must be multiples of 8")
        V = _native.S32Slice
        h, w = hh // 2, ww // 2
        if stem_from_image:
            if isinstance(x, (tuple, list)):
                x = torch.cat([t.float() for t in x], dim=0)
            stem_in = _native.ImgIn(x.float().contiguous())
            self.patches = None
        else:
            if patches is None or tuple(patches.shape[:4]) != (n, h, w, self.w["stem"].kg):
                patches = _native.s32_empty(n, h, w, self.w["stem"].kg, dev)
                _native.stem_patches(x, patches)
            self.patches = patches
            stem_in = V(patches)
        cur = (self._conv1(stem_in, self.w["stem"], (n, h, w)) if self.inorm
               else self._conv_norm(stem_in, self.w["stem"], (n, h, w), "relu"))
        layers = (self.enc.layer1, self.enc.layer2, self.enc.layer3)
        for li, layer in enumerate(layers):
            for bi, blk in enumerate(layer):
                last_of_stage = bi == len(layer) - 1
                out_s2d = last_of_stage and li + 1 < len(layers)
                pre = f"{li}.{bi}."
                if blk.downsample is None:
                    x_in = cur if isinstance(cur, _native.NhwcNormIn) else V(cur)
                    t = self._conv1(x_in, self.w[pre + "conv1"], (n, h, w))
                    cur = self._conv_norm(t, self.w[pre + "conv2"], (n, h, w), "relu", res=x_in, s2d=out_s2d)
                else:
                    h, w = h // 2, w // 2
                    t = self._conv1(V(cur), self.w[pre + "conv1"], (n, h, w))
                    cin = self.w[pre + "down"].kg
                    d = self._conv_norm(V(cur, 0, cin), self.w[pre + "down"], (n, h, w), "none", raw_only=True)
                    res = d if self.inorm else V(d)
                    cur = self._conv_norm(t, self.w[pre + "conv2"], (n, h, w), "relu", res=res, s2d=out_s2d)
                if out_s2d:
                    pass
        head = self.w["head"]
        if split_out:
            out = _native.s32_empty(n, h, w, (head.n + 31) // 32, dev)
            _native.conv_s32(V(cur), head, self._bn(head.n), y0=V(out))
        else:
            out = torch.empty((n, head.n, h, w), device=dev, dtype=torch.float32)
            _native.conv_s32(V(cur), head, self._bn(head.n), f32=out)
        if is_list:
            return torch.split(out, [batch_dim, batch_dim], dim=0)
        return out
```

### torch-optical-flow_amd/methods/raft/model/update.py

```python
from __future__ import annotations

import contextlib
import os
import threading
from typing import Optional, Tuple

import torch
import torch.nn as nn
import torch.nn.functional as F
from torch import Tensor

from optical_flow import _native



CONV_BN = {"c2": 96, "f1": 128, "f2": 64, "mo": 128, "gru": 128, "fh1": 64}
CONV_BN_SIDE = dict(CONV_BN, c2=64, fh1=128)
CONV_BLOCKS = (32, 64, 96, 128)


def parse_block_overrides(var: str, keys) -> dict:
    spec = os.environ.get(var, "")
    out = {}
    for kv in filter(None, (s.strip() for s in spec.split(","))):
        k, sep, v = kv.partition("=")
        if not sep or not v.strip().isdigit():
            raise ValueError(f"{var}={spec!r}: expected comma-separated key=block entries, got {kv!r}")
        key = k.strip()
        if keys is not None and key not in keys:
            raise ValueError(f"{var}={spec!r}: unknown key {key!r} (one of {sorted(keys)})")
        if int(v) not in CONV_BLOCKS:
            raise ValueError(f"{var}={spec!r}: block {v} for {key!r} is not one of {CONV_BLOCKS}")
        out[key] = int(v)
    return out


def _env_choice(var: str, default: str, choices) -> str:
    v = os.environ.get(var, default)
    if v not in choices:
        raise ValueError(f"{var}={v!r}: expected one of {list(choices)}")
    return v


for _bn in (CONV_BN, CONV_BN_SIDE):
    _bn.update(parse_block_overrides("OFLOW_CONV_BN", set(CONV_BN)))
FLOW_HEAD_MODE = _env_choice("OFLOW_FLOW_HEAD_MODE", "fused", ("fused", "tiled", "conv", "col2im"))
CONVF1_FROM_FLOW_MIN_PIXELS = 16384 if _env_choice("OFLOW_CONVF1_FROM_FLOW", "1", ("0", "1")) == "1" else 1 << 62
KSPLIT_LAYERS = frozenset()
KSPLIT_MIN_PIXELS = 16384

class FlowHead(nn.Module):
    def __init__(self, input_dim: int = 128, hidden_dim: int = 256) -> None:
        super().__init__()
        self.conv1 = nn.Conv2d(input_dim, hidden_dim, 3, padding=1)
        self.conv2 = nn.Conv2d(hidden_dim, 2, 3, padding=1)
        self.relu = nn.ReLU(inplace=True)

    def forward(self, x: Tensor) -> Tensor:
        return self.conv2(self.relu(self.conv1(x)))


class SepConvGRU(nn.Module):

    def __init__(self, hidden_dim: int = 128, input_dim: int = 192 + 128) -> None:
        super().__init__()
        cin = hidden_dim + input_dim
        self.convz1 = nn.Conv2d(cin, hidden_dim, (1, 5), padding=(0, 2))
        self.convr1 = nn.Conv2d(cin, hidden_dim, (1, 5), padding=(0, 2))
        self.convq1 = nn.Conv2d(cin, hidden_dim, (1, 5), padding=(0, 2))
        self.convz2 = nn.Conv2d(cin, hidden_dim, (5, 1), padding=(2, 0))
        self.convr2 = nn.Conv2d(cin, hidden_dim, (5, 1), padding=(2, 0))
        self.convq2 = nn.Conv2d(cin, hidden_dim, (5, 1), padding=(2, 0))

    @staticmethod
    def _step(h: Tensor, x: Tensor, convz: nn.Module, convr: nn.Module, convq: nn.Module) -> Tensor:
        hx = torch.cat([h, x], dim=1)
        z = torch.sigmoid(convz(hx))
        r = torch.sigmoid(convr(hx))
        q = torch.tanh(convq(torch.cat([r * h, x], dim=1)))
        return (1 - z) * h + z * q

    def forward(self, h: Tensor, x: Tensor) -> Tensor:
        h = self._step(h, x, self.convz1, self.convr1, self.convq1)
        return self._step(h, x, self.convz2, self.convr2, self.convq2)


class BasicMotionEncoder(nn.Module):

    def __init__(self, corr_levels: int, corr_radius: int) -> None:
        super().__init__()
        corr_planes = corr_levels * (2 * corr_radius + 1) ** 2
        self.convc1 = nn.Conv2d(corr_planes, 256, 1, padding=0)
        self.convc2 = nn.Conv2d(256, 192, 3, padding=1)
        self.convf1 = nn.Conv2d(2, 128, 7, padding=3)
        self.convf2 = nn.Conv2d(128, 64, 3, padding=1)
        self.conv = nn.Conv2d(64 + 192, 128 - 2, 3, padding=1)

    def forward(self, flow: Tensor, corr: Tensor) -> Tensor:
        cor = F.relu(self.convc2(F.relu(self.convc1(corr))))
        flo = F.relu(self.convf2(F.relu(self.convf1(flow))))
        out = F.relu(self.conv(torch.cat([cor, flo], dim=1)))
        return torch.cat([out, flow], dim=1)


class BasicUpdateBlock(nn.Module):

    def __init__(self, corr_levels: int, corr_radius: int, hidden_dim: int = 128) -> None:
        super().__init__()
        self.corr_levels, self.corr_radius = corr_levels, corr_radius
        self.encoder = BasicMotionEncoder(corr_levels, corr_radius)
        self.gru = SepConvGRU(hidden_dim=hidden_dim, input_dim=128 + hidden_dim)
        self.flow_head = FlowHead(hidden_dim, hidden_dim=256)
        self.mask = nn.Sequential(
            nn.Conv2d(128, 256, 3, padding=1), nn.ReLU(inplace=True), nn.Conv2d(256, 64 * 9, 1, padding=0)
        )

    def forward(self, net: Tensor, inp: Tensor, corr: Tensor, flow: Tensor) -> Tuple[Tensor, Tensor, Tensor]:
        motion = self.encoder(flow, corr)
        net = self.gru(net, torch.cat([inp, motion], dim=1))
        delta_flow = self.flow_head(net)
        return net, 0.25 * self.mask(net), delta_flow


class FusedUpdate:

    def __init__(self, block: BasicUpdateBlock, net: Tensor, inp: Tensor) -> None:
        b, ch, h, w = net.shape
        self.block, self.ch, self.ci = block, ch, inp.shape[1]
        enc, gru = block.encoder, block.gru
        cm = enc.conv.out_channels + 2
        total = ch + self.ci + cm
        if gru.convz1.in_channels != total:
            raise RuntimeError("FusedUpdate: unexpected GRU input width")
        self.hx = torch.empty((b, total, h, w), device=net.device, dtype=torch.float32)
        self.rhx = torch.empty_like(self.hx)
        self.hx[:, :ch].copy_(net)
        self.hx[:, ch : ch + self.ci].copy_(inp)
        self.rhx[:, ch : ch + self.ci].copy_(inp)
        self.m0 = ch + self.ci
        self.halves = []
        for tag, pad in (("1", (0, 2)), ("2", (2, 0))):
            cz, cr, cq = (getattr(gru, f"conv{g}{tag}") for g in "zrq")
            wzr = torch.cat([cz.weight, cr.weight], dim=0).contiguous()
            self.halves.append((wzr, cz.bias.contiguous(), cr.bias.contiguous(), cq.weight, cq.bias.contiguous(), pad))

    @staticmethod
    def _conv(x: Tensor, conv: nn.Conv2d) -> Tensor:
        return F.conv2d(x, conv.weight, None, conv.stride, conv.padding, conv.dilation, conv.groups)

    def step(self, corr: Tensor, flow: Tensor, need_mask: bool = True) -> Tuple[Tensor, Optional[Tensor], Tensor]:
        enc, blk = self.block.encoder, self.block
        cor = _native.bias_act_(self._conv(corr, enc.convc1), enc.convc1.bias, "relu")
        cor = _native.bias_act_(self._conv(cor, enc.convc2), enc.convc2.bias, "relu")
        flo = _native.bias_act_(self._conv(flow, enc.convf1), enc.convf1.bias, "relu")
        flo = _native.bias_act_(self._conv(flo, enc.convf2), enc.convf2.bias, "relu")
        out = self._conv(torch.cat([cor, flo], dim=1), enc.conv)
        m0, m1 = self.m0, self.m0 + out.shape[1]
        _native.bias_act_(out, enc.conv.bias, "relu", out=self.hx[:, m0:m1], out2=self.rhx[:, m0:m1])
        self.hx[:, m1:].copy_(flow)
        self.rhx[:, m1:].copy_(flow)
        h = self.hx[:, : self.ch]
        for wzr, bz, br, wq, bq, pad in self.halves:
            zr = F.conv2d(self.hx, wzr, None, 1, pad)
            _native.gru_reset(zr, br, h, self.rhx[:, : self.ch])
            q = F.conv2d(self.rhx, wq, None, 1, pad)
            _native.gru_blend_(zr, bz, q, bq, h)
        net = h.contiguous()
        fh = blk.flow_head
        delta_flow = fh.conv2(_native.bias_act_(self._conv(net, fh.conv1), fh.conv1.bias, "relu"))
        mask = None
        if need_mask:
            m = _native.bias_act_(self._conv(net, blk.mask[0]), blk.mask[0].bias, "relu")
            mask = _native.bias_act_(self._conv(m, blk.mask[2]), blk.mask[2].bias, "none", scale=0.25)
        return net, mask, delta_flow


class FusedLookup:

    __slots__ = ("pyr", "coords", "radius")

    def __init__(self, pyr, coords: Tensor, radius: int) -> None:
        self.pyr, self.coords, self.radius = pyr, coords, radius


_SIDE_STREAMS = {}


def _side_stream(device: torch.device, slot: int = 0) -> "torch.cuda.Stream":
    dev = torch.device(device)
    owner = torch.cuda.current_stream(dev).stream_id
    key = (dev.index, owner, slot)
    if key not in _SIDE_STREAMS:
        _SIDE_STREAMS[key] = torch.cuda.Stream(device=device)
    return _SIDE_STREAMS[key]


_CAPTURE = threading.local()


@contextlib.contextmanager
def capturing(device: torch.device):
    depth = _CAPTURE.__dict__.setdefault("depth", {})
    idx = torch.device(device).index
    depth[idx] = depth.get(idx, 0) + 1
    try:
        yield
    finally:
        depth[idx] -= 1


def capture_active(device: Optional[torch.device] = None) -> bool:
    idx = torch.device(device).index if device is not None else torch.cuda.current_device()
    if _CAPTURE.__dict__.get("depth", {}).get(idx, 0) > 0:
        return True
    return torch.cuda.is_current_stream_capturing()


def _module_device(module: nn.Module) -> Optional[torch.device]:
    for p in module.parameters():
        return p.device
    return None


def cached_pack(module: nn.Module, key, build):
    dev = _module_device(module)
    on_gpu = dev is not None and dev.type == "cuda"
    cache = module.__dict__.get("_split_weights")
    if cache is not None and cache[0] == key:
        if cache[2] is not None and on_gpu and not capture_active(dev):
            torch.cuda.current_stream(dev).wait_event(cache[2])
        return cache[1]
    if on_gpu:
        with torch.cuda.device(dev):
            w = build()
            ev = torch.cuda.Event()
            ev.record(torch.cuda.current_stream(dev))
    else:
        w, ev = build(), None
    module.__dict__["_split_weights"] = (key, w, ev)
    return w


def tensor_key(q: Tensor):
    return (q.data_ptr(), -1 if q.is_inference() else q._version)


def _weights_key(block: nn.Module):
    return tuple(tensor_key(q) for q in block.parameters())


class SplitUpdate:

    def __init__(self, block: BasicUpdateBlock, cnet_out: Tensor, hdim: int, side_slot: int = 0,
                 fuse_c1: bool = True, flow_head_pixels: Optional[int] = None, side_owner=None) -> None:
        b, c, h, w = cnet_out.shape
        enc, gru = block.encoder, block.gru
        cdim = c - hdim
        if (hdim, cdim, enc.conv.out_channels, gru.convz1.in_channels) != (128, 128, 126, 384):
            raise RuntimeError("SplitUpdate: supports the RAFT (large) update block only")
        dev = cnet_out.device
        self.block, self.shape = block, (b, h, w)
        px = b * h * w if flow_head_pixels is None else int(flow_head_pixels)
        self.flow_head_fma = px < _native.FLOW_HEAD2_MAX_PIXELS
        self.f1_from_flow = px >= CONVF1_FROM_FLOW_MIN_PIXELS
        self.ks = _native.KSplit(b, h, w, dev) if KSPLIT_LAYERS and px >= KSPLIT_MIN_PIXELS else None
        self.ks_mo = self.ks if "mo" in KSPLIT_LAYERS else None
        self.ks_q = self.ks if "q" in KSPLIT_LAYERS else None
        S = _native.s32_empty
        self.hx = S(b, h, w, 8, dev)
        self.rhx = S(b, h, w, 8, dev)
        levels, radius = block.corr_levels, block.corr_radius
        self.corr_ch = levels * (2 * radius + 1) ** 2
        self.corr_f32 = None
        self.c1 = S(b, h, w, 8, dev)
        self.cf = S(b, h, w, 8, dev)
        self.pm = None if self.f1_from_flow else S(b, h, w, 4, dev)
        self.f1 = S(b, h, w, 4, dev)
        self.fh = S(b, h, w, 8, dev)
        self.fh2y = None
        self.flow_head_mode = getattr(block, "flow_head_mode", FLOW_HEAD_MODE)
        self.fused_head = self.flow_head_mode == "fused" and not self.flow_head_fma
        self.fhy = _native.flow_head_partial_empty(b, h, w, dev) if self.fused_head else None
        self.flow_for = None
        self.hm = torch.empty((b * h * w, hdim), device=dev, dtype=torch.float32)
        self.z = torch.empty_like(self.hm)
        V = _native.S32Slice
        _native.pack_s32(cnet_out[:, :hdim], "tanh", V(self.hx, 0, 4), nhwc=self.hm)
        inp = S(b, h, w, 4, dev)
        _native.pack_s32(cnet_out[:, hdim:], "relu", V(inp))
        self.w = self._weights(block)
        self.gx = []
        for tag in ("1", "2"):
            gx = torch.empty((b * h * w, 3 * hdim), device=dev, dtype=torch.float32)
            _native.conv_s32(V(inp), self.w["inp" + tag], 128, nhwc=gx)
            self.gx.append(gx)
        self.fuse_c1 = fuse_c1 and "c1L" in self.w
        self.streams = getattr(block, "split_streams", True)
        self.side_stream = None
        if self.streams:
            if side_owner is None:
                self.side_stream = _side_stream(dev, side_slot)
            else:
                with torch.cuda.stream(side_owner):
                    self.side_stream = _side_stream(dev, side_slot)

    @staticmethod
    def _weights(block: BasicUpdateBlock):
        return cached_pack(block, _weights_key(block), lambda: SplitUpdate._pack(block))

    @staticmethod
    def _pack(block: BasicUpdateBlock):
        enc, gru, fh = block.encoder, block.gru, block.flow_head
        CW = _native.ConvWeights
        w = {
            "c1": CW(enc.convc1.weight, enc.convc1.bias, 256),
            "c2": CW(enc.convc2.weight, enc.convc2.bias, 192),
            "f1": CW(enc.convf1.weight, enc.convf1.bias, 128, patches=True),
            "f2": CW(enc.convf2.weight, enc.convf2.bias, 64),
            "mo": CW(enc.conv.weight, enc.conv.bias, 128),
            "fh1": CW(fh.conv1.weight, fh.conv1.bias, 256),
            "fh2": CW(fh.conv2.weight, fh.conv2.bias, 32),
            "fh2T": CW(fh.conv2.weight.detach().float().permute(2, 3, 0, 1).reshape(18, -1, 1, 1), None, 32),
            "fh2_bias": fh.conv2.bias.detach().float().contiguous(),
            "fh2_f32": (fh.conv2.weight.detach().float().contiguous(), fh.conv2.bias.detach().float().contiguous()),
            "fh2_tiled": (_native.flow_head2_tiled_weights(fh.conv2.weight), fh.conv2.bias.detach().float().contiguous()),
            "fh2_fused": _native.flow_head_fused_weights(fh.conv2.weight),
            "m1": CW(block.mask[0].weight, block.mask[0].bias, 256),
            "m2": CW(block.mask[2].weight, block.mask[2].bias, 576),
        }
        if block.corr_radius in (3, 4):
            w["c1L"] = _native.convc1_level_weights(enc.convc1, block.corr_levels, block.corr_radius)
        for tag in ("1", "2"):
            cz, cr, cq = (getattr(gru, f"conv{g}{tag}") for g in "zrq")
            hmf = lambda wt: torch.cat([wt[:, :128], wt[:, 256:]], dim=1)
            w["zr" + tag] = CW(hmf(torch.cat([cz.weight, cr.weight])), None, 256)
            w["q" + tag] = CW(hmf(cq.weight), None, 128)
            w["inp" + tag] = CW(torch.cat([cz.weight, cr.weight, cq.weight])[:, 128:256],
                                torch.cat([cz.bias, cr.bias, cq.bias]), 384)
        return w

    def step(self, corr_fn, coords1: Tensor, need_mask: bool, mask_out: Optional[Tensor] = None) -> Optional[Tensor]:
        return self.update(self.lookup(corr_fn, coords1), coords1, need_mask, mask_out)

    def lookup_rows(self, coords1: Tensor) -> Tensor:
        if self.corr_f32 is None:
            b, h, wd = self.shape
            self.corr_f32 = torch.empty((b * h * wd, self.corr_ch), device=coords1.device, dtype=torch.float32)
        return self.corr_f32

    def fusable(self, corr_fn) -> bool:
        return self.fuse_c1 and getattr(corr_fn, "_tiled", None) is not None and corr_fn.radius in (3, 4)

    def lookup(self, corr_fn, coords1: Tensor):
        if self.fusable(corr_fn):
            return FusedLookup(corr_fn._tiled, coords1, corr_fn.radius)
        b, h, wd = self.shape
        corr_fn.lookup_nhwc(coords1, self.lookup_rows(coords1))
        return _native.F32In(self.corr_f32, b, h, wd)

    def _convc1(self, corr_in) -> None:
        if isinstance(corr_in, FusedLookup):
            _native.corr_lookup_convc1(corr_in.pyr, corr_in.coords, corr_in.radius, self.w["c1L"], _native.S32Slice(self.c1))
        else:
            _native.conv_s32(corr_in, self.w["c1"], 128, "relu", y0=_native.S32Slice(self.c1))

    def update(self, corr_in, coords1: Tensor, need_mask: bool, mask_out: Optional[Tensor] = None) -> Optional[Tensor]:
        V, conv, w = _native.S32Slice, _native.conv_s32, self.w
        b, h, wd = self.shape
        main = torch.cuda.current_stream(coords1.device)
        side = self.side_stream if self.streams else None
        bns = CONV_BN_SIDE if side is not None else CONV_BN
        f1_in = V(self.pm) if self.pm is not None else _native.FlowIn(coords1)
        fused = self.fused_head and coords1.is_contiguous()
        flow_key = (coords1.data_ptr(), tuple(coords1.shape))
        prep = self.pm is not None or not fused or self.flow_for != flow_key
        self.flow_for = None
        if side is not None:
            side.wait_stream(main)
            with torch.cuda.stream(side):
                if prep:
                    _native.flow_prep(coords1, self.pm, (V(self.hx), 254), (V(self.rhx), 254))
                conv(f1_in, w["f1"], bns["f1"], "relu", y0=V(self.f1))
                conv(V(self.f1), w["f2"], bns["f2"], "relu", y0=V(self.cf, 6, 2))
            self._convc1(corr_in)
            conv(V(self.c1), w["c2"], bns["c2"], "relu", y0=V(self.cf, 0, 6))
            main.wait_stream(side)
        else:
            if prep:
                _native.flow_prep(coords1, self.pm, (V(self.hx), 254), (V(self.rhx), 254))
            self._convc1(corr_in)
            conv(V(self.c1), w["c2"], bns["c2"], "relu", y0=V(self.cf, 0, 6))
            conv(f1_in, w["f1"], bns["f1"], "relu", y0=V(self.f1))
            conv(V(self.f1), w["f2"], bns["f2"], "relu", y0=V(self.cf, 6, 2))
        conv(V(self.cf), w["mo"], bns["mo"], "relu", y0=V(self.hx, 4, 4), y1=V(self.rhx, 4, 4), ksplit=self.ks_mo)
        for tag, gx in zip(("1", "2"), self.gx):
            conv(V(self.hx), w["zr" + tag], bns["gru"], epilogue=1, y0=V(self.rhx, 0, 4), gru_h=self.hm, gru_z=self.z,
                 addend=gx[:, :256])
            conv(V(self.rhx), w["q" + tag], bns["gru"], epilogue=2, y0=V(self.hx, 0, 4), gru_h=self.hm, gru_z=self.z,
                 addend=gx[:, 256:], ksplit=self.ks_q)
        net = V(self.hx, 0, 4)
        if fused:
            _native.conv_s32_flow_head(net, w["fh1"], bns["fh1"], w["fh2_fused"], self.fhy)
            _native.flow_head_finish(self.fhy, w["fh2_bias"], coords1, (V(self.hx), 254), (V(self.rhx), 254))
            self.flow_for = flow_key
            return self._mask(net, coords1, mask_out) if need_mask else None
        conv(net, w["fh1"], bns["fh1"], "relu", y0=V(self.fh))
        if self.flow_head_fma and coords1.is_contiguous():
            _native.flow_head2(V(self.fh), *w["fh2_f32"], coords1)
        elif self.flow_head_mode == "tiled" and coords1.is_contiguous():
            _native.flow_head2_tiled(V(self.fh), *w["fh2_tiled"], coords1)
        elif self.flow_head_mode == "col2im" and coords1.is_contiguous():
            if self.fh2y is None:
                self.fh2y = torch.empty((b, 18, h, wd), device=coords1.device, dtype=torch.float32)
            conv(V(self.fh), w["fh2T"], 32, f32=self.fh2y)
            _native.flow_head_col2im(self.fh2y, w["fh2_bias"], coords1)
        else:
            conv(V(self.fh), w["fh2"], 32, f32=coords1, f32_accumulate=True)
        return self._mask(net, coords1, mask_out) if need_mask else None

    def _mask(self, net, coords1: Tensor, mask_out: Optional[Tensor]) -> Tensor:
        V, conv, w = _native.S32Slice, _native.conv_s32, self.w
        b, h, wd = self.shape
        mask = mask_out if mask_out is not None else torch.empty((b, 576, h, wd), device=coords1.device, dtype=torch.float32)
        conv(net, w["m1"], 128, "relu", y0=V(self.fh))
        conv(V(self.fh), w["m2"], 64, out_scale=0.25, f32=mask)
        return mask
```

### torch-optical-flow_amd/optical_flow/_native.py

```python
from __future__ import annotations

import ctypes
import os
from typing import List, Optional, Sequence

import torch

from . import _ops

_LIB_PATH = os.environ.get(
    "OFLOW_LIB", os.path.join(os.path.dirname(os.path.abspath(__file__)), "_lib", "liboflow_hip.so")
)
ABI_VERSION = 1
MAX_LEVELS = 8
MAX_RADIUS = 7
FLOW_HEAD2_MAX_PIXELS = 16384
E_TINY = -4

INTERP = {"bilinear": 0, "nearest": 1, "bicubic": 2}
PADDING = {"zeros": 0, "border": 1, "reflection": 2}

SYMBOLS = (
    "oflow_abi_version",
    "oflow_status_string",
    "oflow_corr_pyramid_dims",
    "oflow_corr_pyramid_f32",
    "oflow_corr_lookup_f32",
    "oflow_corr_tiled_level_floats",
    "oflow_corr_pyramid_tiled_f32",
    "oflow_corr_lookup_tiled_f32",
    "oflow_corr_untile_f32",
    "oflow_grid_warp_f32",
    "oflow_grid_sample_f32",
    "oflow_corr_otf_prepare_f16",
    "oflow_corr_lookup_otf_f16",
    "oflow_bias_act_f32",
    "oflow_gru_reset_f32",
    "oflow_gru_blend_f32",
    "oflow_conv_s32",
    "oflow_pack_s32_f32",
    "oflow_flow_prep_s32",
    "oflow_conv_s32_ex",
    "oflow_stem_patches_s32",
    "oflow_norm_stats_finalize",
    "oflow_norm_apply_s32",
    "oflow_convex_upsample_f32",
    "oflow_conv_s32_ex2",
    "oflow_corr_lookup_tiled_nhwc_f32",
    "oflow_corr_lookup_backward_f32",
    "oflow_corr_pyramid_grad_combine_f32",
    "oflow_flow_stats_f32",
    "oflow_flow2rgb_f32",
    "oflow_flow_pack_f32",
    "oflow_corr_lookup_convc1_s32",
    "oflow_corr_pyramid_tiled_s32",
    "oflow_flow_head2_s32",
    "oflow_flow_head2_tiled_s32",
    "oflow_conv_s32_ex3",
    "oflow_conv_s32_ex4",
    "oflow_conv_s32_ex5",
    "oflow_normalize_images_f32",
    "oflow_replicate_pad_f32",
    "oflow_corr_fmap_grad_f32",
    "oflow_grid_warp_backward_f32",
    "oflow_grid_sample_backward_f32",
    "oflow_set_range_flag",
    "oflow_range_flag_exchange",
    "oflow_flow_head_col2im_f32",
    "oflow_conv_s32_ex6",
    "oflow_flow_head_finish_f32",
    "oflow_timing_event_create",
    "oflow_timing_event_destroy",
    "oflow_timing_event_record",
    "oflow_timing_event_elapsed_ms",
    "oflow_flow_error_stats_f32",
    "oflow_sequence_loss_f32",
    "oflow_sequence_loss_backward_f32",
)

_lib = None
_recorder = None
_flops = None


def set_flop_counter(counter):
    global _flops
    _flops = counter


def _count(exec_f16: int, useful: int, fma: int = 0) -> None:
    _flops["exec_f16"] = _flops.get("exec_f16", 0) + exec_f16
    _flops["useful"] = _flops.get("useful", 0) + useful
    _flops["fma_f32"] = _flops.get("fma_f32", 0) + fma


def set_event_recorder(recorder):
    global _recorder
    _recorder = recorder


class TimingEvent:

    __slots__ = ("ev",)

    def __init__(self):
        ev = ctypes.c_void_p()
        _check(load().oflow_timing_event_create(ctypes.byref(ev)), "timing_event_create")
        self.ev = ev

    def record(self, stream: "torch.cuda.Stream") -> None:
        _check(load().oflow_timing_event_record(self.ev, ctypes.c_void_p(stream.cuda_stream), 1), "timing_event_record")

    def elapsed_time(self, end: "TimingEvent") -> float:
        ms = ctypes.c_float()
        _check(load().oflow_timing_event_elapsed_ms(self.ev, end.ev, ctypes.byref(ms)), "timing_event_elapsed_ms")
        return float(ms.value)

    def __del__(self):
        try:
            if _lib is not None and self.ev:
                _lib.oflow_timing_event_destroy(self.ev)
        except Exception:
            pass


_TIMED_DEFAULT = ("corr_lookup", "corr_lookup_convc1", "corr_pyramid", "corr_lookup_otf", "corr_otf_prepare", "grid_warp")


class _Timed:
    __slots__ = ("what", "stream", "ev0")

    def __init__(self, what: str, device: torch.device):
        self.what = what
        on = _recorder is not None and (what in _TIMED_DEFAULT or _recorder.get("*", False))
        self.stream = torch.cuda.current_stream(device) if on else None
        self.ev0 = None

    def __enter__(self):
        if self.stream is not None:
            self.ev0 = TimingEvent() if _recorder.get("_native") else torch.cuda.Event(enable_timing=True)
            self.ev0.record(self.stream)
        return self

    def __exit__(self, *exc):
        if self.stream is not None and exc[0] is None and _recorder is not None:
            ev1 = TimingEvent() if _recorder.get("_native") else torch.cuda.Event(enable_timing=True)
            ev1.record(self.stream)
            _recorder.setdefault(self.what, []).append((self.ev0, ev1))
        return False


def library_path() -> str:
    return _LIB_PATH


def load() -> ctypes.CDLL:
    global _lib
    if _lib is not None:
        return _lib
    if not os.path.exists(_LIB_PATH):
        raise RuntimeError(
            f"liboflow_hip.so not found at {_LIB_PATH}: build it with `make -C torch-optical-flow_amd/csrc` "
            "(or __graft_entry__.build()); the MI355X path has no CPU fallback"
        )
    lib = ctypes.CDLL(_LIB_PATH)
    P, I, F = ctypes.c_void_p, ctypes.c_int, ctypes.c_float
    IP = ctypes.POINTER(ctypes.c_int)
    PP = ctypes.POINTER(ctypes.c_void_p)
    lib.oflow_abi_version.restype = I
    lib.oflow_abi_version.argtypes = []
    lib.oflow_status_string.restype = ctypes.c_char_p
    lib.oflow_status_string.argtypes = [I]
    lib.oflow_corr_pyramid_dims.restype = I
    lib.oflow_corr_pyramid_dims.argtypes = [I, I, I, IP, IP]
    lib.oflow_corr_pyramid_f32.restype = I
    lib.oflow_corr_pyramid_f32.argtypes = [P, P, I, I, I, I, I, PP, P]
    lib.oflow_corr_lookup_f32.restype = I
    lib.oflow_corr_lookup_f32.argtypes = [PP, IP, IP, I, P, I, I, I, I, P, P]
    lib.oflow_corr_tiled_level_floats.restype = ctypes.c_longlong
    lib.oflow_corr_tiled_level_floats.argtypes = [I, I]
    lib.oflow_corr_pyramid_tiled_f32.restype = I
    lib.oflow_corr_pyramid_tiled_f32.argtypes = [P, P, I, I, I, I, I, PP, P]
    lib.oflow_corr_lookup_tiled_f32.restype = I
    lib.oflow_corr_lookup_tiled_f32.argtypes = [PP, IP, IP, I, P, I, I, I, I, P, P]
    lib.oflow_corr_untile_f32.restype = I
    lib.oflow_corr_untile_f32.argtypes = [P, P, ctypes.c_longlong, I, I, P]
    lib.oflow_grid_warp_f32.restype = I
    lib.oflow_grid_warp_f32.argtypes = [P, P, I, I, I, I, I, I, I, P, P]
    lib.oflow_grid_sample_f32.restype = I
    lib.oflow_grid_sample_f32.argtypes = [P, P, I, I, I, I, I, I, I, I, I, P, P]
    lib.oflow_corr_otf_prepare_f16.restype = I
    lib.oflow_corr_otf_prepare_f16.argtypes = [P, P, I, I, I, I, I, P, PP, P, P]
    L = ctypes.c_longlong
    lib.oflow_bias_act_f32.restype = I
    lib.oflow_bias_act_f32.argtypes = [P, L, P, P, L, P, L, I, I, I, I, F, P]
    lib.oflow_gru_reset_f32.restype = I
    lib.oflow_gru_reset_f32.argtypes = [P, L, P, P, L, P, L, I, I, I, P]
    lib.oflow_gru_blend_f32.restype = I
    lib.oflow_gru_blend_f32.argtypes = [P, L, P, P, L, P, P, L, I, I, I, P]
    lib.oflow_conv_s32.restype = I
    lib.oflow_conv_s32.argtypes = [P, L, I, P, I, P, P, I, I, I, I, I, I, I, I, I, F, P, L, P, L, P, L, L, I, P, P, I, P]
    lib.oflow_conv_s32_ex.restype = I
    lib.oflow_conv_s32_ex.argtypes = [P, L, I, P, I, P, P, I, I, I, I, I, I, I, I, I, F, P, L, P, L, P, L, L, I, P, P, I,
                                      P, I, P, P, L, I, I, P]
    lib.oflow_stem_patches_s32.restype = I
    lib.oflow_stem_patches_s32.argtypes = [P, I, I, I, I, P, I, P]
    lib.oflow_norm_stats_finalize.restype = I
    lib.oflow_norm_stats_finalize.argtypes = [P, I, I, I, I, ctypes.c_double, P, P, P]
    lib.oflow_norm_apply_s32.restype = I
    lib.oflow_norm_apply_s32.argtypes = [P, I, I, I, I, P, P, I, I, P, L, P, P, P, I, I, P, L, P]
    lib.oflow_pack_s32_f32.restype = I
    lib.oflow_pack_s32_f32.argtypes = [P, L, I, I, I, I, I, I, P, L, P, L, P, I, P]
    lib.oflow_flow_prep_s32.restype = I
    lib.oflow_flow_prep_s32.argtypes = [P, I, I, I, P, P, L, P, L, P]
    lib.oflow_corr_lookup_otf_f16.restype = I
    lib.oflow_corr_lookup_otf_f16.argtypes = [P, PP, IP, IP, I, P, I, I, I, I, I, P, P]
    lib.oflow_conv_s32_ex2.restype = I
    lib.oflow_conv_s32_ex2.argtypes = list(lib.oflow_conv_s32_ex.argtypes[:-1]) + [I, P, P, P]
    lib.oflow_conv_s32_ex3.restype = I
    lib.oflow_conv_s32_ex3.argtypes = list(lib.oflow_conv_s32_ex2.argtypes[:-1]) + [P, L, P]
    lib.oflow_conv_s32_ex4.restype = I
    lib.oflow_normalize_images_f32.restype = I
    lib.oflow_normalize_images_f32.argtypes = [P, P, L, P, P, P]
    lib.oflow_replicate_pad_f32.restype = I
    lib.oflow_replicate_pad_f32.argtypes = [P, P, I, L, I, I, I, I, I, I, P]
    lib.oflow_conv_s32_ex4.argtypes = list(lib.oflow_conv_s32_ex3.argtypes[:-1]) + [P, P]
    lib.oflow_conv_s32_ex5.restype = I
    lib.oflow_conv_s32_ex5.argtypes = list(lib.oflow_conv_s32_ex4.argtypes[:-1]) + [P, P, L, P]
    lib.oflow_corr_lookup_backward_f32.restype = I
    lib.oflow_corr_lookup_backward_f32.argtypes = [P, P, I, I, I, I, PP, IP, IP, I, P]
    lib.oflow_corr_pyramid_grad_combine_f32.restype = I
    lib.oflow_corr_pyramid_grad_combine_f32.argtypes = [PP, IP, IP, I, L, P]
    lib.oflow_corr_lookup_tiled_nhwc_f32.restype = I
    lib.oflow_corr_lookup_tiled_nhwc_f32.argtypes = [PP, IP, IP, I, P, I, I, I, I, P, I, P]
    lib.oflow_convex_upsample_f32.restype = I
    lib.oflow_flow_head2_s32.restype = I
    lib.oflow_flow_head2_s32.argtypes = [P, ctypes.c_longlong, I, P, P, I, I, I, P, P]
    lib.oflow_flow_head2_tiled_s32.restype = I
    lib.oflow_flow_head2_tiled_s32.argtypes = [P, ctypes.c_longlong, I, P, P, I, I, I, P, P]
    lib.oflow_corr_pyramid_tiled_s32.restype = I
    lib.oflow_corr_pyramid_tiled_s32.argtypes = [P, P, I, I, I, I, I, PP, P]
    lib.oflow_corr_lookup_convc1_s32.restype = I
    lib.oflow_corr_lookup_convc1_s32.argtypes = [PP, IP, IP, I, P, I, I, I, I, P, P, P, P, ctypes.c_longlong, P]
    lib.oflow_convex_upsample_f32.argtypes = [P, P, I, I, I, P, P]
    lib.oflow_flow_stats_f32.restype = I
    lib.oflow_flow_stats_f32.argtypes = [P, I, I, I, I, F, F, I, P, P]
    lib.oflow_flow2rgb_f32.restype = I
    lib.oflow_flow2rgb_f32.argtypes = [P, I, I, I, I, I, F, F, I, I, F, P, P, P]
    lib.oflow_flow_pack_f32.restype = I
    lib.oflow_flow_pack_f32.argtypes = [P, I, I, I, I, I, P, P]
    lib.oflow_set_range_flag.restype = I
    lib.oflow_set_range_flag.argtypes = [P]
    lib.oflow_range_flag_exchange.restype = I
    lib.oflow_range_flag_exchange.argtypes = [P, P, P]
    lib.oflow_timing_event_create.restype = I
    lib.oflow_timing_event_create.argtypes = [ctypes.POINTER(ctypes.c_void_p)]
    lib.oflow_timing_event_destroy.restype = I
    lib.oflow_timing_event_destroy.argtypes = [P]
    lib.oflow_timing_event_record.restype = I
    lib.oflow_timing_event_record.argtypes = [P, P, I]
    lib.oflow_timing_event_elapsed_ms.restype = I
    lib.oflow_timing_event_elapsed_ms.argtypes = [P, P, ctypes.POINTER(ctypes.c_float)]
    lib.oflow_flow_head_col2im_f32.restype = I
    lib.oflow_flow_head_col2im_f32.argtypes = [P, P, I, I, I, P, P]
    lib.oflow_conv_s32_ex6.restype = I
    lib.oflow_conv_s32_ex6.argtypes = list(lib.oflow_conv_s32_ex5.argtypes[:-1]) + [P, P, I, P]
    lib.oflow_flow_head_finish_f32.restype = I
    lib.oflow_flow_head_finish_f32.argtypes = [P, I, P, I, I, I, P, P, L, P, L, P]
    FP = ctypes.POINTER(F)
    lib.oflow_flow_error_stats_f32.restype = I
    lib.oflow_flow_error_stats_f32.argtypes = [P, L, L, L, P, L, L, L, P, I, L, L, I, I, I, F, F, F, P, P, P, P]
    lib.oflow_sequence_loss_f32.restype = I
    lib.oflow_sequence_loss_f32.argtypes = [PP, I, FP, P, P, I, I, I, I, F, P, P, P, P]
    lib.oflow_sequence_loss_backward_f32.restype = I
    lib.oflow_sequence_loss_backward_f32.argtypes = [P, PP, PP, I, FP, P, P, I, I, I, I, F, P]
    v = lib.oflow_abi_version()
    if v != ABI_VERSION:
        raise RuntimeError(f"liboflow_hip.so ABI version {v}, expected {ABI_VERSION}: rebuild the library")
    _ops.load()
    _lib = lib
    return lib


def ops():
    if _lib is None:
        load()
    return torch.ops.oflow


def _run(what: str, device: torch.device, op, *args):
    if _recorder is None:
        return op(*args)
    with _Timed(what, device):
        return op(*args)


def _tensor(t, name: str, what: str) -> torch.Tensor:
    if not isinstance(t, torch.Tensor):
        raise TypeError(f"{what}: {name} must be a torch.Tensor")
    return t


def _no_grad_input(t: torch.Tensor, name: str, what: str) -> None:
    if t.requires_grad and torch.is_grad_enabled():
        raise RuntimeError(
            f"{what}: {name} requires grad; this layout is inference-only (no backward): use CorrBlock's canonical "
            "pyramid (corr_pyramid / corr_lookup have autograd), or run under torch.no_grad()"
        )


def _check(status: int, what: str) -> None:
    if status == 0:
        return
    msg = load().oflow_status_string(status).decode()
    if status == E_TINY:
        raise ValueError(f"{what}: {msg}")
    raise RuntimeError(f"{what} failed ({status}): {msg}")


def _gpu_f32(t: torch.Tensor, name: str, what: str) -> torch.Tensor:
    if not isinstance(t, torch.Tensor):
        raise TypeError(f"{what}: {name} must be a torch.Tensor")
    if t.device.type != "cuda":
        raise RuntimeError(
            f"{what}: {name} is on {t.device}; this MI355X build runs only on ROCm GPU tensors (no CPU fallback)"
        )
    if t.requires_grad and torch.is_grad_enabled():
        raise RuntimeError(
            f"{what}: {name} requires grad; this entry point is an inference layout with no autograd formula: use "
            "CorrBlock / optical_flow.warp (native backward kernels), or run under torch.no_grad() / "
            "torch.inference_mode(), or detach the input"
        )
    if t.dtype != torch.float32:
        t = t.float()
    return t.contiguous()


def _stream(device: torch.device) -> ctypes.c_void_p:
    return ctypes.c_void_p(torch.cuda.current_stream(device).cuda_stream)


def pyramid_dims(h: int, w: int, num_levels: int):
    hs = (ctypes.c_int * MAX_LEVELS)()
    ws = (ctypes.c_int * MAX_LEVELS)()
    _check(load().oflow_corr_pyramid_dims(h, w, num_levels, hs, ws), "corr_pyramid_dims")
    return [(hs[i], ws[i]) for i in range(num_levels)]


def corr_pyramid(fmap1: torch.Tensor, fmap2: torch.Tensor, num_levels: int = 4) -> List[torch.Tensor]:
    f1, f2 = _tensor(fmap1, "fmap1", "corr_pyramid"), _tensor(fmap2, "fmap2", "corr_pyramid")
    return list(_run("corr_pyramid", f1.device, ops().corr_pyramid, f1, f2, int(num_levels)))


class TiledPyramid:

    __slots__ = ("levels", "dims", "queries")

    def __init__(self, levels, dims, queries):
        self.levels, self.dims, self.queries = levels, dims, queries

    def batch_slice(self, b0: int, b1: int) -> "TiledPyramid":
        hw = self.dims[0][0] * self.dims[0][1]
        return TiledPyramid([t[b0 * hw : b1 * hw] for t in self.levels], self.dims, (b1 - b0) * hw)

    def untile(self, l: int) -> torch.Tensor:
        hl, wl = self.dims[l]
        src = self.levels[l]
        out = torch.empty((self.queries, 1, hl, wl), device=src.device, dtype=torch.float32)
        if out.numel():
            with torch.cuda.device(src.device):
                _check(load().oflow_corr_untile_f32(src.data_ptr(), out.data_ptr(), self.queries, hl, wl, _stream(src.device)), "untile")
        return out


def corr_pyramid_tiled(fmap1: torch.Tensor, fmap2: torch.Tensor, num_levels: int = 4) -> TiledPyramid:
    what = "corr_pyramid"
    f1, f2 = _tensor(fmap1, "fmap1", what), _tensor(fmap2, "fmap2", what)
    _no_grad_input(f1, "fmap1", what)
    _no_grad_input(f2, "fmap2", what)
    levels = list(_run(what, f1.device, ops().corr_pyramid_tiled, f1, f2, int(num_levels)))
    return TiledPyramid(levels, pyramid_dims(f1.shape[2], f1.shape[3], num_levels), int(levels[0].shape[0]))


def corr_pyramid_tiled_s32(f1: torch.Tensor, f2: torch.Tensor, num_levels: int = 4) -> TiledPyramid:
    what = "corr_pyramid"
    for t in (f1, f2):
        if t.dtype != torch.float16 or t.dim() != 6 or tuple(t.shape[-2:]) != (2, 32) or not t.is_contiguous():
            raise RuntimeError(f"{what}: S32 feature maps must be contiguous fp16 (B, H, W, G, 2, 32)")
        if t.device.type != "cuda":
            raise RuntimeError(f"{what}: S32 feature maps must be on the GPU (no CPU fallback)")
    if f1.shape != f2.shape or f1.device != f2.device:
        raise RuntimeError(f"{what}: feature maps differ in shape or device")
    b, h, w, g = (int(v) for v in f1.shape[:4])
    dims = pyramid_dims(h, w, num_levels)
    lib = load()
    per_q = [int(lib.oflow_corr_tiled_level_floats(hl, wl)) for hl, wl in dims]
    q = b * h * w
    store = torch.empty((q * sum(per_q),), device=f1.device, dtype=torch.float32)
    levels, off = [], 0
    for n in per_q:
        levels.append(store[off * q : (off + n) * q].view(q, n))
        off += n
    ptrs = (ctypes.c_void_p * MAX_LEVELS)(*[t.data_ptr() for t in levels])
    if _flops is not None:
        _count(3 * 2 * b * (h * w) ** 2 * g * 32, 2 * b * (h * w) ** 2 * g * 32)
    with torch.cuda.device(f1.device), _Timed(what, f1.device):
        _check(lib.oflow_corr_pyramid_tiled_s32(f1.data_ptr(), f2.data_ptr(), b, g * 32, h, w, int(num_levels), ptrs,
                                                _stream(f1.device)), what)
    return TiledPyramid(levels, dims, q)


def corr_lookup_tiled(pyr: TiledPyramid, coords: torch.Tensor, radius: int) -> torch.Tensor:
    co = _tensor(coords, "coords", "corr_lookup")
    _no_grad_input(co, "coords", "corr_lookup")
    return _run("corr_lookup", co.device, ops().corr_lookup_tiled, pyr.levels, co, int(radius))


def corr_lookup(levels: Sequence[torch.Tensor], coords: torch.Tensor, radius: int) -> torch.Tensor:
    co = _tensor(coords, "coords", "corr_lookup")
# ... 270 lines not shown

    def channel_ptr(self, c: int) -> int:
        return self.ptr + (c // 32) * 128 + (c % 32) * 2

    @property
    def bhw(self):
        return tuple(int(v) for v in self.t.shape[:3])

    @property
    def device(self):
        return self.t.device


class F32In:

    __slots__ = ("raw", "bhw")
    in_format = 2

    def __init__(self, raw: torch.Tensor, b: int, h: int, w: int):
        if raw.dtype != torch.float32 or not raw.is_contiguous() or raw.shape[0] != b * h * w or raw.shape[1] % 4:
            raise RuntimeError("F32In: raw must be contiguous fp32 [B*H*W, C], C % 4 == 0")
        self.raw, self.bhw = raw, (int(b), int(h), int(w))

    @property
    def ptr(self) -> int:
        return self.raw.data_ptr()

    @property
    def ps(self) -> int:
        return int(self.raw.shape[1]) * 4

    @property
    def ng(self) -> int:
        return (int(self.raw.shape[1]) + 31) // 32

    @property
    def device(self):
        return self.raw.device


class ImgIn:

    __slots__ = ("raw", "bhw")
    in_format = 3

    def __init__(self, img: torch.Tensor):
        if img.dtype != torch.float32 or img.dim() != 4 or img.shape[1] != 3 or not img.is_contiguous():
            raise RuntimeError("ImgIn: the image must be contiguous fp32 (B, 3, H, W)")
        b, _, hh, ww = img.shape
        if hh % 2 or ww % 2:
            raise RuntimeError("ImgIn: H and W must be even")
        self.raw, self.bhw = img, (int(b), int(hh) // 2, int(ww) // 2)

    @property
    def ptr(self) -> int:
        return self.raw.data_ptr()

    @property
    def ps(self) -> int:
        return 0

    @property
    def ng(self) -> int:
        return 5

    @property
    def device(self):
        return self.raw.device


class FlowIn:

    __slots__ = ("raw", "bhw")
    in_format = 4

    def __init__(self, coords: torch.Tensor):
        if coords.dtype != torch.float32 or coords.dim() != 4 or coords.shape[1] != 2 or not coords.is_contiguous():
            raise RuntimeError("FlowIn: coords must be contiguous fp32 (B, 2, H, W)")
        b, _, hh, ww = coords.shape
        self.raw, self.bhw = coords, (int(b), int(hh), int(ww))

    @property
    def ptr(self) -> int:
        return self.raw.data_ptr()

    @property
    def ps(self) -> int:
        return 0

    @property
    def ng(self) -> int:
        return 4

    @property
    def device(self):
        return self.raw.device


class NhwcNormIn:

    __slots__ = ("raw", "bhw", "scale", "shift")
    in_format = 1

    def __init__(self, raw: torch.Tensor, b: int, h: int, w: int, scale: torch.Tensor, shift: torch.Tensor):
        c = raw.shape[1]
        if raw.dtype != torch.float32 or not raw.is_contiguous() or raw.shape[0] != b * h * w or c % 32:
            raise RuntimeError("NhwcNormIn: raw must be contiguous fp32 [B*H*W, C], C % 32 == 0")
        for t in (scale, shift):
            if t.dtype != torch.float32 or not t.is_contiguous() or t.numel() != b * c:
                raise RuntimeError("NhwcNormIn: scale / shift must be contiguous fp32 [B, C]")
        self.raw, self.bhw, self.scale, self.shift = raw, (int(b), int(h), int(w)), scale, shift

    @property
    def ptr(self) -> int:
        return self.raw.data_ptr()

    @property
    def ps(self) -> int:
        return int(self.raw.shape[1]) * 4

    @property
    def ng(self) -> int:
        return int(self.raw.shape[1]) // 32

    @property
    def device(self):
        return self.raw.device


def s32_empty(b: int, h: int, w: int, groups: int, device, zero: bool = False) -> torch.Tensor:
    f = torch.zeros if zero else torch.empty
    return f((b, h, w, groups, 2, 32), device=device, dtype=torch.float16)


def s32_from_f32(x: torch.Tensor, groups: int = -1) -> torch.Tensor:
    b, c, h, w = x.shape
    g = (c + 31) // 32 if groups < 0 else groups
    v = torch.zeros((b, h, w, g * 32), device=x.device, dtype=torch.float32)
    v[..., :c] = x.permute(0, 2, 3, 1)
    hi = v.half()
    lo = (v - hi.float()).half()
    return torch.stack([hi.view(b, h, w, g, 32), lo.view(b, h, w, g, 32)], dim=4).contiguous()


def s32_to_f32(t: torch.Tensor, channels: int = -1) -> torch.Tensor:
    b, h, w, g = t.shape[:4]
    v = (t[:, :, :, :, 0].float() + t[:, :, :, :, 1].float()).reshape(b, h, w, g * 32)
    c = g * 32 if channels < 0 else channels
    return v[..., :c].permute(0, 3, 1, 2).contiguous()


class ConvWeights:

    __slots__ = ("pack", "wscale", "bias", "n", "n_pad", "kh", "kw", "kg", "layout", "cin", "_frag")

    def __init__(self, weight: torch.Tensor, bias, n_pad: int, patches: bool = False):
        w = weight.detach().float()
        if patches:
            n, c, kh, kw = w.shape
            w = w.permute(0, 2, 3, 1).reshape(n, kh * kw * c, 1, 1)
        n, c, kh, kw = w.shape
        if n_pad < n:
            raise RuntimeError("ConvWeights: n_pad < out channels")
        amax = w.abs().amax(dim=(1, 2, 3))
        e = torch.where(amax > 0, torch.ceil(torch.log2(amax)), torch.zeros_like(amax)).clamp(-100, 100)
        scale = torch.exp2(14.0 - e)
        ws = w * scale.view(-1, 1, 1, 1)
        kg = (c + 31) // 32
        t = kh * kw
        full = torch.zeros((n_pad, kg * 32, t), device=w.device, dtype=torch.float32)
        full[:n, :c] = ws.reshape(n, c, t)
        full = full.view(n_pad, kg, 32, t).permute(1, 3, 0, 2).contiguous()
        hi = full.half()
        lo = (full - hi.float()).half()
        self.pack = torch.stack([hi, lo], dim=3).contiguous()
        inv = torch.ones(n_pad, device=w.device, dtype=torch.float32)
        inv[:n] = 1.0 / scale
        self.wscale = inv
        self.bias = None if bias is None else bias.detach().float().contiguous()
        self.n, self.n_pad, self.kh, self.kw, self.kg = n, n_pad, kh, kw, kg
        self.cin = c
        self.layout = "conv"
        self._frag = None
        if t > 1 and n_pad % 32 == 0:
            self.frag()

    def frag(self) -> torch.Tensor:
        if self._frag is None:
            if self.layout != "conv" or self.n_pad % 32:
                raise RuntimeError("ConvWeights.frag: needs a conv-layout pack with n_pad a multiple of 32")
            kg, t = self.pack.shape[:2]
            f = self.pack.reshape(kg, t, self.n_pad // 32, 32, 2, 2, 2, 8)
            self._frag = f.permute(0, 1, 2, 5, 4, 6, 3, 7).contiguous()
        return self._frag


def convc1_level_weights(conv: torch.nn.Conv2d, num_levels: int, radius: int) -> "ConvWeights":
    kk = (2 * radius + 1) ** 2
    g = (kk + 31) // 32
    w = conv.weight.detach().float()
    if tuple(w.shape[1:]) != (num_levels * kk, 1, 1):
        raise RuntimeError(f"convc1_level_weights: expected a 1x1 conv over {num_levels * kk} channels, got {tuple(w.shape)}")
    wp = w.new_zeros((w.shape[0], num_levels * g * 32, 1, 1))
    for l in range(num_levels):
        wp[:, l * g * 32 : l * g * 32 + kk] = w[:, l * kk : (l + 1) * kk]
    cw = ConvWeights(wp, conv.bias, w.shape[0])
    lg = cw.pack.shape[0]
    frag = cw.pack.reshape(lg, 4, 2, 32, 2, 2, 2, 8)
    cw.pack = frag.permute(0, 1, 2, 5, 4, 6, 3, 7).contiguous()
    cw.layout = "convc1_frag"
    cw.cin = num_levels * kk
    return cw


def corr_lookup_convc1(pyr: "TiledPyramid", coords: torch.Tensor, radius: int, cw: "ConvWeights", y: "S32Slice") -> None:
    what = "corr_lookup_convc1"
    co = _gpu_f32(coords, "coords", what)
    b, two, h, w = co.shape
    if two != 2 or b * h * w != pyr.queries:
        raise RuntimeError(f"{what}: coords (B, 2, H, W) must cover the pyramid's {pyr.queries} queries")
    kk = (2 * radius + 1) ** 2
    if (cw.layout != "convc1_frag" or cw.n != 256 or cw.n_pad != 256 or cw.kh * cw.kw != 1
            or cw.kg != len(pyr.levels) * ((kk + 31) // 32)):
        raise RuntimeError(f"{what}: weights must be convc1_level_weights of this pyramid / radius")
    if y.ng != 8 or y.bhw != (b, h, w) or y.device != co.device:
        raise RuntimeError(f"{what}: destination must be an 8-group S32 slice of shape ({b}, {h}, {w})")
    n = len(pyr.levels)
    ptrs = (ctypes.c_void_p * MAX_LEVELS)(*[t.data_ptr() for t in pyr.levels])
    hs = (ctypes.c_int * MAX_LEVELS)(*[d[0] for d in pyr.dims])
    ws = (ctypes.c_int * MAX_LEVELS)(*[d[1] for d in pyr.dims])
    if _flops is not None:
        _count(3 * 2 * b * h * w * 256 * cw.kg * 32, 2 * b * h * w * 256 * cw.cin)
    with torch.cuda.device(co.device), _Timed(what, co.device):
        _check(
            load().oflow_corr_lookup_convc1_s32(
                ptrs, hs, ws, n, co.data_ptr(), b, h, w, int(radius), cw.pack.data_ptr(), cw.wscale.data_ptr(),
                cw.bias.data_ptr() if cw.bias is not None else None, y.ptr, y.ps, _stream(co.device),
            ),
            what,
        )


def conv_tiles(h: int, w: int) -> int:
    return ((h + 3) // 4) * ((w + 31) // 32)


class KSplit:

    def __init__(self, b: int, h: int, w: int, device, block_n: int = 128, blocks: int = 1) -> None:
        self.tiles = b * conv_tiles(h, w) * blocks
        self.block_n = block_n
        self.slab = torch.empty(self.tiles * 128 * block_n, device=device, dtype=torch.float32)
        self.ctr = torch.zeros(2 * self.tiles, device=device, dtype=torch.int32)


def conv_s32(x: S32Slice, cw: ConvWeights, block_n: int, act: str = "none", out_scale: float = 1.0, y0=None, y1=None,
             f32=None, f32_accumulate: bool = False, epilogue: int = 0, gru_h=None, gru_z=None, nhwc=None, stats=None,
             res=None, res_act: str = "none", s2d: bool = False, addend=None, ksplit: "KSplit" = None) -> None:
    what = "conv_s32"
    if CHECK_RANGE:
        _range_check(x, f"{what} {cw.kh}x{cw.kw}")
    if x.ng != cw.kg:
        raise RuntimeError(f"{what}: input has {x.ng} groups, weights expect {cw.kg}")
    b, h, w = x.bhw
    nin = isinstance(x, NhwcNormIn)
    in_format = getattr(x, "in_format", 0)
    hw_out = (h // 2, w // 2) if s2d else (h, w)
    for d in (y0, y1):
        if d is not None and (tuple(d.t.shape[:3]) != (b, *hw_out) or d.t.device != x.device):
            raise RuntimeError(f"{what}: destination shape/device mismatch")
    if res is not None and (tuple(res.t.shape[:3]) != (b, h, w) or res.ng * 32 < cw.n):
        raise RuntimeError(f"{what}: residual shape mismatch")
    fp, fbs, fcs = 0, 0, 0
    if f32 is not None:
        if f32.dtype != torch.float32 or f32.dim() != 4 or tuple(f32.shape[2:]) != (h, w) or f32.shape[0] != b:
            raise RuntimeError(f"{what}: fp32 destination must be (B, C, H, W) fp32")
        if f32.stride(3) != 1 or f32.stride(2) != w or f32.shape[1] < cw.n and epilogue == 0:
            raise RuntimeError(f"{what}: fp32 destination planes must be contiguous with >= N channels")
        fp, fbs, fcs = f32.data_ptr(), f32.stride(0), f32.stride(1)
    if nhwc is not None and (nhwc.dtype != torch.float32 or not nhwc.is_contiguous() or nhwc.numel() != b * h * w * cw.n):
        raise RuntimeError(f"{what}: nhwc destination must be contiguous fp32 [P, {cw.n}]")
    if stats is not None and (stats.dtype != torch.float32 or stats.numel() < b * conv_tiles(h, w) * cw.n_pad * 3):
        raise RuntimeError(f"{what}: stats partials buffer too small")
    gh = gz = 0
    gch = 0
    if epilogue:
        gch = cw.n // 2 if epilogue == 1 else cw.n
        for tt in (gru_h, gru_z):
            if tt is None or tt.dtype != torch.float32 or not tt.is_contiguous() or tt.numel() != b * h * w * gch:
                raise RuntimeError(f"{what}: GRU state tensors must be contiguous fp32 [P, {gch}]")
        gh, gz = gru_h.data_ptr(), gru_z.data_ptr()
    ap, aps = 0, 0
    if addend is not None:
        if (not epilogue or addend.dtype != torch.float32 or addend.dim() != 2 or addend.stride(1) != 1
                or addend.shape[0] != b * h * w or addend.shape[1] < cw.n or addend.stride(0) % 4
                or addend.data_ptr() % 16 or addend.device != x.device):
            raise RuntimeError(f"{what}: addend must be a GRU-epilogue fp32 [P, >= {cw.n}] view with 16-B aligned rows")
        ap, aps = addend.data_ptr(), addend.stride(0)
    dev = x.device
    wf = (cw.frag().data_ptr() if CONV_BREG and (int(block_n) == 128 or (CONV_BREG64 and int(block_n) == 64)
                                                 or (CONV_BREG32 and int(block_n) == 32))
          and cw.kh * cw.kw > 1 and not nin
          and in_format == 0 and cw.layout == "conv" else None)
    if _flops is not None:
        taps, p_out = cw.kh * cw.kw, b * h * w
        n_exec = -(-cw.n_pad // int(block_n)) * int(block_n)
        _count(3 * 2 * p_out * n_exec * cw.kg * 32 * taps, 2 * p_out * cw.n * cw.cin * taps)
    ks_slab = ks_ctr = None
    ks_tiles = 0
    if ksplit is not None and wf is not None:
        if ksplit.slab.device != dev or ksplit.block_n < int(block_n):
            raise RuntimeError(f"{what}: split-K scratch on another device or for narrower channel blocks")
        ks_slab, ks_ctr = ksplit.slab.data_ptr(), ksplit.ctr.data_ptr()
        ks_tiles = ksplit.tiles * (ksplit.block_n // int(block_n))
    with torch.cuda.device(dev), _Timed(f"conv{cw.kh}x{cw.kw}", dev):
        _check(
            load().oflow_conv_s32_ex5(
                x.ptr, x.ps, cw.kg, cw.pack.data_ptr(), cw.n_pad, cw.wscale.data_ptr(),
                cw.bias.data_ptr() if cw.bias is not None else None, cw.n, b, h, w, cw.kh, cw.kw, int(block_n),
                int(epilogue), ACT[act], float(out_scale), y0.ptr if y0 is not None else None, y0.ps if y0 is not None else 0,
                y1.ptr if y1 is not None else None, y1.ps if y1 is not None else 0, fp or None, fbs, fcs,
                int(bool(f32_accumulate)), gh or None, gz or None, gch,
                nhwc.data_ptr() if nhwc is not None else None, cw.n,
                stats.data_ptr() if stats is not None else None,
                res.ptr if res is not None else None, res.ps if res is not None else 0, ACT[res_act], int(bool(s2d)),
                in_format, x.scale.data_ptr() if nin else None, x.shift.data_ptr() if nin else None,
                ap or None, aps, wf, ks_slab, ks_ctr, ks_tiles, _stream(dev),
            ),
            what,
        )


def flow_head2(x: "S32Slice", weight: torch.Tensor, bias: torch.Tensor, coords: torch.Tensor) -> None:
    what = "flow_head2"
    b, h, w = x.bhw
    if weight.dtype != torch.float32 or not weight.is_contiguous() or tuple(weight.shape) != (2, x.ng * 32, 3, 3):
        raise RuntimeError(f"{what}: weight must be contiguous fp32 (2, {x.ng * 32}, 3, 3)")
    if bias is None or bias.dtype != torch.float32 or tuple(bias.shape) != (2,):
        raise RuntimeError(f"{what}: bias must be fp32 (2,)")
    if coords.dtype != torch.float32 or not coords.is_contiguous() or tuple(coords.shape) != (b, 2, h, w):
        raise RuntimeError(f"{what}: coords must be contiguous fp32 ({b}, 2, {h}, {w})")
    if _flops is not None:
        fl = 2 * b * h * w * 2 * x.ng * 32 * 9
        _count(0, fl, fl)
    with torch.cuda.device(coords.device), _Timed("conv3x3", coords.device):
        _check(load().oflow_flow_head2_s32(x.ptr, x.ps, x.ng, weight.data_ptr(), bias.data_ptr(), b, h, w,
                                           coords.data_ptr(), _stream(coords.device)), what)


def flow_head2_tiled_weights(weight: torch.Tensor) -> torch.Tensor:
    o, c = weight.shape[:2]
    if o != 2 or c % 32 or tuple(weight.shape[2:]) != (3, 3):
        raise RuntimeError("flow_head2_tiled_weights: weight must be (2, C, 3, 3) with C a multiple of 32")
    w = weight.detach().float().reshape(2, c // 32, 8, 4, 3, 3)
    return w.permute(1, 2, 4, 5, 0, 3).contiguous()


def flow_head2_tiled(x: "S32Slice", wr: torch.Tensor, bias: torch.Tensor, coords: torch.Tensor) -> None:
    what = "flow_head2_tiled"
    b, h, w = x.bhw
    if wr.dtype != torch.float32 or not wr.is_contiguous() or wr.numel() != 2 * x.ng * 32 * 9 or wr.data_ptr() % 16:
        raise RuntimeError(f"{what}: wr must be flow_head2_tiled_weights of a (2, {x.ng * 32}, 3, 3) weight")
    if bias is None or bias.dtype != torch.float32 or tuple(bias.shape) != (2,):
        raise RuntimeError(f"{what}: bias must be fp32 (2,)")
    if coords.dtype != torch.float32 or not coords.is_contiguous() or tuple(coords.shape) != (b, 2, h, w):
        raise RuntimeError(f"{what}: coords must be contiguous fp32 ({b}, 2, {h}, {w})")
    if _flops is not None:
        fl = 2 * b * h * w * 2 * x.ng * 32 * 9
        _count(0, fl, fl)
    with torch.cuda.device(coords.device), _Timed("conv3x3", coords.device):
        _check(load().oflow_flow_head2_tiled_s32(x.ptr, x.ps, x.ng, wr.data_ptr(), bias.data_ptr(), b, h, w,
                                                 coords.data_ptr(), _stream(coords.device)), what)


def flow_head_col2im(y: torch.Tensor, bias: torch.Tensor, coords: torch.Tensor) -> None:
    what = "flow_head_col2im"
    b, _, h, w = coords.shape
    if coords.dtype != torch.float32 or not coords.is_contiguous() or coords.shape[1] != 2 or coords.device.type != "cuda":
        raise RuntimeError(f"{what}: coords must be contiguous fp32 (B, 2, H, W) on the GPU")
    if y.dtype != torch.float32 or not y.is_contiguous() or tuple(y.shape) != (b, 18, h, w) or y.device != coords.device:
        raise RuntimeError(f"{what}: y must be contiguous fp32 ({b}, 18, {h}, {w})")
    if bias is None or bias.dtype != torch.float32 or tuple(bias.shape) != (2,) or bias.device != coords.device:
        raise RuntimeError(f"{what}: bias must be fp32 (2,) on the coords' device")
    with torch.cuda.device(coords.device), _Timed("flow_head_col2im", coords.device):
        _check(load().oflow_flow_head_col2im_f32(y.data_ptr(), bias.data_ptr(), b, h, w, coords.data_ptr(),
                                                 _stream(coords.device)), what)


FLOW_HEAD_SLABS = 4


def flow_head_fused_weights(weight: torch.Tensor) -> torch.Tensor:
    if tuple(weight.shape) != (2, 64 * FLOW_HEAD_SLABS, 3, 3):
        raise RuntimeError(f"flow_head_fused_weights: weight must be (2, {64 * FLOW_HEAD_SLABS}, 3, 3)")
    return weight.detach().float().permute(1, 2, 3, 0).reshape(FLOW_HEAD_SLABS, 64, 18).contiguous()


def flow_head_partial_empty(b: int, h: int, w: int, device) -> torch.Tensor:
    return torch.empty((FLOW_HEAD_SLABS, b, 18, h, w), device=device, dtype=torch.float32)


def conv_s32_flow_head(x: "S32Slice", cw: "ConvWeights", block_n: int, w2r: torch.Tensor, partial) -> None:
    what = "conv_s32_flow_head"
    if x.ng != cw.kg:
        raise RuntimeError(f"{what}: input has {x.ng} groups, weights expect {cw.kg}")
    b, h, w = x.bhw
    dev = x.device
    if (w2r.dtype != torch.float32 or not w2r.is_contiguous() or tuple(w2r.shape[1:]) != (64, 18) or w2r.device != dev):
        raise RuntimeError(f"{what}: w2r must be flow_head_fused_weights(conv2.weight) on the input's device")
    slabs, pp = 0, None
    if partial is not None:
        if (partial.dtype != torch.float32 or not partial.is_contiguous() or partial.dim() != 5
                or tuple(partial.shape[1:]) != (b, 18, h, w) or partial.device != dev):
            raise RuntimeError(f"{what}: partial must be contiguous fp32 (slabs, {b}, 18, {h}, {w}) on the input's device")
        slabs, pp = int(partial.shape[0]), partial.data_ptr()
    if w2r.shape[0] != FLOW_HEAD_SLABS:
        slabs = -1
    wf = cw.frag().data_ptr() if int(block_n) == 128 and cw.layout == "conv" else None
    if _flops is not None:
        n_exec = -(-cw.n_pad // int(block_n)) * int(block_n)
        _count(3 * 2 * b * h * w * n_exec * cw.kg * 32 * 9, 2 * b * h * w * cw.n * cw.cin * 9)
        fl = 2 * b * h * w * 2 * cw.n * 9
        _count(0, fl, fl)
    with torch.cuda.device(dev), _Timed("conv3x3", dev):
        _check(
            load().oflow_conv_s32_ex6(
                x.ptr, x.ps, cw.kg, cw.pack.data_ptr(), cw.n_pad, cw.wscale.data_ptr(),
                cw.bias.data_ptr() if cw.bias is not None else None, cw.n, b, h, w, cw.kh, cw.kw, int(block_n),
                3, ACT["relu"], 1.0, None, 0, None, 0, None, 0, 0, 0, None, None, 0, None, cw.n, None, None, 0, 0, 0,
                0, None, None, None, 0, wf, None, None, 0, w2r.data_ptr(), pp, slabs, _stream(dev),
            ),
            what,
        )


def flow_head_finish(partial: torch.Tensor, bias: torch.Tensor, coords: torch.Tensor, flow0=None, flow1=None) -> None:
    what = "flow_head_finish"
    if (coords.dtype != torch.float32 or coords.dim() != 4 or coords.shape[1] != 2 or not coords.is_contiguous()
            or coords.device.type != "cuda"):
        raise RuntimeError(f"{what}: coords must be contiguous fp32 (B, 2, H, W) on the GPU")
    b, _, h, w = coords.shape
    if (partial.dtype != torch.float32 or not partial.is_contiguous() or partial.dim() != 5
            or tuple(partial.shape[1:]) != (b, 18, h, w) or partial.device != coords.device):
        raise RuntimeError(f"{what}: partial must be contiguous fp32 (slabs, {b}, 18, {h}, {w})")
    if bias is None or bias.dtype != torch.float32 or tuple(bias.shape) != (2,) or bias.device != coords.device:
        raise RuntimeError(f"{what}: bias must be fp32 (2,) on the coords' device")
    for fl in (flow0, flow1):
        if fl is not None and (fl[0].bhw != (b, h, w) or fl[0].device != coords.device):
            raise RuntimeError(f"{what}: flow destination shape/device mismatch")
    f0 = (flow0[0].channel_ptr(flow0[1]), flow0[0].ps) if flow0 is not None else (None, 0)
    f1 = (flow1[0].channel_ptr(flow1[1]), flow1[0].ps) if flow1 is not None else (None, 0)
    with torch.cuda.device(coords.device), _Timed("flow_head_finish", coords.device):
        _check(load().oflow_flow_head_finish_f32(partial.data_ptr(), int(partial.shape[0]), bias.data_ptr(), b, h, w,
                                                 coords.data_ptr(), f0[0], f0[1], f1[0], f1[1],
                                                 _stream(coords.device)), what)


def stem_patches(img: torch.Tensor, out: torch.Tensor) -> torch.Tensor:
    x = _gpu_f32(img, "image", "stem_patches")
    b, c, h, w = x.shape
    if out.dtype != torch.float16 or tuple(out.shape[:3]) != (b, (h + 1) // 2, (w + 1) // 2):
        raise RuntimeError("stem_patches: output must be S32 (B, ceil(H/2), ceil(W/2), G, 2, 32)")
    with torch.cuda.device(x.device), _Timed("stem_patches", x.device):
        _check(load().oflow_stem_patches_s32(x.data_ptr(), b, c, h, w, out.data_ptr(), int(out.shape[3]), _stream(x.device)), "stem_patches")
    return out


def norm_stats(partials: torch.Tensor, b: int, tiles: int, n_pad: int, c: int, eps: float):
    alpha = torch.empty((b, c), device=partials.device, dtype=torch.float32)
    beta = torch.empty_like(alpha)
    with torch.cuda.device(partials.device):
        _check(
            load().oflow_norm_stats_finalize(partials.data_ptr(), b, tiles, n_pad, c, float(eps), alpha.data_ptr(), beta.data_ptr(), _stream(partials.device)),
            "norm_stats",
        )
    return alpha, beta


def norm_apply(x: torch.Tensor, shape, alpha, beta, act: str, y: S32Slice, res=None, res_raw=None, res_act: str = "none",
               s2d: bool = False, res_raw_relu: bool = False) -> None:
    b, c, h, w = shape
    mode, rp, rps = 0, None, 0
    x2 = a2 = b2 = None
    if res is not None:
        mode, rp, rps = 1, res.ptr, res.ps
# ... 95 lines not shown
```

Measured before the change: 466.0 image-pairs/s.

## Add grouped two-problem conv launch with tap-skipping for space-to-depth stride-2 convs

Adds a grouped conv entry point that runs up to two conv problems in one launch, with the block-y index choosing the problem. For 2x2 space-to-depth convs it compiles masked K-loops that visit only the (group, tap) steps whose weights are nonzero, so the structurally zero taps of the stride-2 3x3 and 1x1 shortcut are not multiplied. The encoder's stride-2 head uses the tap-skipping path by default, and can optionally fuse the downsample shortcut into the same launch. Motion-encoder c2/f2 grouping is added behind a flag that is off by default. The masked loop adds code size and per-launch host work to classify live taps, and its schedule differs from the tuned generic loop.

```diff
diff --git a/include/oflow.h b/include/oflow.h
--- a/include/oflow.h
+++ b/include/oflow.h
@@ -169,6 +169,26 @@
                        long long addend_pixel_stride, const void* d_wfrag, float* d_ksplit_slab,
                        unsigned* d_ksplit_ctr, long long ksplit_tiles, const float* d_fh_weights, float* d_fh_partial,
                        int fh_slabs, void* stream);
+typedef struct oflow_conv_problem {
+  const void* d_x;
+  long long x_pixel_stride;
+  int in_groups;
+  const void* d_wpack;
+  int n_pad;
+  const float* d_wscale;
+  const float* d_bias;
+  int N;
+  int B, H, W;
+  const unsigned char* step_live;
+  int activation;
+  float out_scale;
+  void* d_y0;
+  long long y0_pixel_stride;
+  float* d_nhwc;
+  int nhwc_pixel_stride;
+  float* d_stats;
+} oflow_conv_problem;
+int oflow_conv_s32_group(const oflow_conv_problem* problems, int count, int kh, int kw, int block_n, void* stream);
 int oflow_stem_patches_s32(const float* d_img, int B, int C, int H, int W, void* d_out, int out_groups, void* stream);
 int oflow_norm_stats_finalize(const float* d_partials, int B, int tiles, int n_pad, int C, double eps, float* d_alpha,
                               float* d_beta, void* stream);
diff --git a/torch-optical-flow_amd/csrc/conv_s32.hip b/torch-optical-flow_amd/csrc/conv_s32.hip
--- a/torch-optical-flow_amd/csrc/conv_s32.hip
+++ b/torch-optical-flow_amd/csrc/conv_s32.hip
@@ -1,4 +1,6 @@
 #include "oflow_internal.h"
+
+#include <type_traits>
 
 namespace oflow {
 namespace {
@@ -87,6 +89,34 @@
 constexpr int kImgC = 3, kImgK = 7, kImgRows = (kTY - 1) * 2 + kImgK, kImgCols = (kTX - 1) * 2 + kImgK;
 constexpr int kImgHalf = (kImgCols + 1) / 2, kImgPitch = 2 * kImgHalf, kImgPlane = kImgRows * kImgPitch;
 
+constexpr unsigned kTapsS2D3x3 = 0xFAC8u, kTapsS2D1x1 = 0x0008u;
+struct TapSteps {
+  int n, ng;
+  int sid[64];
+  int gidx[64];
+  bool last[64];
+  int grp[16];
+};
+constexpr TapSteps tap_steps(unsigned tp, int gq) {
+  TapSteps s{};
+  for (int q = 0; q < 4; ++q) {
+    const unsigned m = (tp >> (4 * q)) & 15u;
+    if (m == 0u) continue;
+    for (int gi = 0; gi < gq; ++gi) {
+      const int g = q * gq + gi;
+      for (int t = 0; t < 4; ++t)
+        if ((m >> t) & 1u) {
+          s.sid[s.n] = g * 4 + t;
+          s.gidx[s.n] = s.ng;
+          s.last[s.n] = (m >> (t + 1)) == 0u;
+          ++s.n;
+        }
+      s.grp[s.ng++] = g;
+    }
+  }
+  return s;
+}
+
 __device__ __forceinline__ float sigmoid_hw(float v) {
   return __builtin_amdgcn_rcpf(1.0f + __builtin_amdgcn_exp2f(v * -1.4426950408889634f));
 }
@@ -179,8 +209,24 @@
   }
 }
 
-template <int KH, int KW, int BN, int WM, int WN, int EPI, int TY = kTY, int AIN = kInS32, bool BREG = false, int BD = 1>
-__global__ __launch_bounds__(64 * WM * WN, WM * WN == 8 ? 1 : 2) void conv_s32_kernel(ConvArgs a) {
+template <class T, class... R>
+__device__ __forceinline__ const T& first_arg(const T& t, const R&...) { return t; }
+struct GroupArgs {
+  ConvArgs p[2];
+  int split;
+  int var[2];
+};
+template <int KH, int KW, int BN, int WM, int WN, int EPI, int TY = kTY, int AIN = kInS32, bool BREG = false, int BD = 1,
+          unsigned TP0 = 0u, unsigned TP1 = 0u, int KGS = 0, class... Tail>
+__global__ __launch_bounds__(64 * WM * WN, WM * WN == 8 ? 1 : 2) void conv_s32_kernel(ConvArgs a, Tail... tail) {
+  int cb0 = 0, variant = -1;
+  if constexpr (sizeof...(Tail) != 0) {
+    const GroupArgs& g = first_arg(tail...);
+    const int sel = static_cast<int>(blockIdx.y) >= g.split ? 1 : 0;
+    a = g.p[sel];
+    cb0 = sel ? g.split : 0;
+    variant = g.var[sel];
+  }
   constexpr int NTH = 64 * WM * WN;
   constexpr int T = KH * KW;
   constexpr int BM = TY * kTX;
@@ -255,7 +301,10 @@
     }
   } else {
     tile = blockIdx.x;
-    cblk = blockIdx.y;
+    if constexpr (sizeof...(Tail) != 0)
+      cblk = static_cast<int>(blockIdx.y) - cb0;
+    else
+      cblk = blockIdx.y;
   }
   const int tx0 = (tile % a.tiles_x) * kTX;
   tile /= a.tiles_x;
@@ -396,6 +445,25 @@
       BL[nt_] = *reinterpret_cast<const half8*>(row_ + ((clo_ ^ bswz(n_)) << 4));                                    \
     }                                                                                                                \
   }
+#define OFLOW_READ_OPS_T(AH, AL, BH, BL, TAP, PAR, S_)                                                               \
+  {                                                                                                                  \
+    const int t_ = (TAP), ky_ = t_ / KW, kx_ = t_ - ky_ * KW;                                                         \
+    const uint8_t* bufA_ = sA;                                                                                        \
+    const uint8_t* bufB_ = sB + (PAR) * B_BYTES;                                                                      \
+    const int chi_ = 2 * (S_) + hh, clo_ = 4 + 2 * (S_) + hh;                                                        \
+    _Pragma("unroll") for (int mt_ = 0; mt_ < MT; ++mt_) {                                                           \
+      const int p_ = (wm * MT + mt_ + ky_) * HX + r + kx_;                                                           \
+      const uint8_t* row_ = bufA_ + p_ * RSA;                                                                        \
+      AH[mt_] = *reinterpret_cast<const half8*>(row_ + ((chi_ ^ aswz(p_)) << 4));                                    \
+      AL[mt_] = *reinterpret_cast<const half8*>(row_ + ((clo_ ^ aswz(p_)) << 4));                                    \
+    }                                                                                                                \
+    _Pragma("unroll") for (int nt_ = 0; nt_ < NT; ++nt_) {                                                           \
+      const int n_ = wn * (BN / WN) + nt_ * 32 + r;                                                                  \
+      const uint8_t* row_ = bufB_ + n_ * RSB;                                                                        \
+      BH[nt_] = *reinterpret_cast<const half8*>(row_ + ((chi_ ^ bswz(n_)) << 4));                                    \
+      BL[nt_] = *reinterpret_cast<const half8*>(row_ + ((clo_ ^ bswz(n_)) << 4));                                    \
+    }                                                                                                                \
+  }
 #define OFLOW_MFMAS(AH, AL, BH, BL)                                                                                  \
   if (!OFLOW_ABL(2)) _Pragma("unroll") for (int mt = 0; mt < MT; ++mt)                                               \
     _Pragma("unroll") for (int nt = 0; nt < NT; ++nt) {                                                              \
@@ -613,6 +681,59 @@
 #undef OFLOW_READ_A
 #undef OFLOW_MFMAS_R
   } else {
+  bool masked_done = false;
+  if constexpr (TP0 != 0u || TP1 != 0u) {
+    static_assert(KH == 2 && KW == 2 && AIN == kInS32 && !ADB && KGS % 4 == 0 && KGS >= 4 && KGS <= 16,
+                  "tap patterns: 2x2 convs on S32 input, four equal quarters of the input groups");
+    auto masked_loop = [&](auto tpc) __attribute__((always_inline)) {
+      static constexpr TapSteps ts = tap_steps(decltype(tpc)::value, KGS / 4);
+      constexpr int L = ts.n, NG = ts.ng;
+      static_assert(L >= 1 && NG >= 1, "a pattern with no live step");
+      u32x4 rbr[BD][BPER];
+      u32x4 rar[1][APER];
+      OFLOW_LOAD_B(rbr[0], ts.sid[0]);
+      OFLOW_LOAD_A(rar[0], ts.grp[0]);
+      OFLOW_WRITE_A(rar[0], 0, ts.grp[0]);
+      OFLOW_WRITE_B(rbr[0], 0);
+#pragma unroll
+      for (int d = 1; d <= BD; ++d) OFLOW_LOAD_B(rbr[d % BD], ts.sid[d < L ? d : L - 1]);
+      OFLOW_LOAD_A(rar[0], ts.grp[NG > 1 ? 1 : 0]);
+      __syncthreads();
+      half8 xah[MT], xal[MT], xbh[NT], xbl[NT];
+      half8 yah[MT], yal[MT], ybh[NT], ybl[NT];
+      OFLOW_READ_OPS_T(xah, xal, xbh, xbl, ts.sid[0] % T, 0, 0);
+#pragma unroll
+      for (int i = 0; i < L; ++i) {
+        u32x4 (&rb)[BPER] = rbr[(i + 1) % BD];
+        OFLOW_WRITE_B(rb, (i + 1) & 1);
+        OFLOW_LOAD_B(rb, ts.sid[i + 1 + BD < L ? i + 1 + BD : L - 1]);
+        OFLOW_READ_OPS_T(yah, yal, ybh, ybl, ts.sid[i] % T, i & 1, 1);
+        OFLOW_MFMAS(xah, xal, xbh, xbl);
+        if (ts.last[i]) {
+          const int k = ts.gidx[i];
+          __syncthreads();
+          OFLOW_WRITE_A(rar[0], 0, ts.grp[k + 1 < NG ? k + 1 : k]);
+          OFLOW_LOAD_A(rar[0], ts.grp[k + 2 < NG ? k + 2 : NG - 1]);
+        }
+        __syncthreads();
+        OFLOW_READ_OPS_T(xah, xal, xbh, xbl, ts.sid[i + 1 < L ? i + 1 : L - 1] % T, (i + 1) & 1, 0);
+        OFLOW_MFMAS(yah, yal, ybh, ybl);
+      }
+    };
+    if constexpr (TP0 != 0u) {
+      if (variant == 0) {
+        masked_loop(std::integral_constant<unsigned, TP0>{});
+        masked_done = true;
+      }
+    }
+    if constexpr (TP1 != 0u) {
+      if (variant == 1) {
+        masked_loop(std::integral_constant<unsigned, TP1>{});
+        masked_done = true;
+      }
+    }
+  }
+  if ((TP0 == 0u && TP1 == 0u) || !masked_done) {
   u32x4 rbr[BD][BPER];
   u32x4 rar[ADB ? BD : 1][APER];
   OFLOW_LOAD_B(rbr[0], 0);
@@ -662,8 +783,10 @@
     }
   }
   }
+  }
 #undef OFLOW_MFMAS
 #undef OFLOW_READ_OPS
+#undef OFLOW_READ_OPS_T
 #undef OFLOW_LOAD_A
 #undef OFLOW_WRITE_A
 #undef OFLOW_LOAD_B
@@ -1415,6 +1538,67 @@
   return dispatch_conv(a, kh, kw, block_n, epilogue, static_cast<hipStream_t>(stream));
 }
 
+namespace oflow {
+namespace {
+
+int live_variant(const unsigned char* live, int in_groups, int taps, unsigned tp0, unsigned tp1, int kgs) {
+  if (live == nullptr || taps != 4 || in_groups != kgs || kgs == 0) return -1;
+  const int gq = in_groups / 4;
+  unsigned need = 0u;
+  for (int g = 0; g < in_groups; ++g)
+    for (int t = 0; t < 4; ++t)
+      if (live[g * 4 + t]) need |= 1u << (4 * (g / gq) + t);
+  if (need == 0u) return -1;
+  if (tp0 != 0u && (need & ~tp0) == 0u && (tp1 == 0u || (need & ~tp1) != 0u || tp0 == tp1)) return 0;
+  if (tp1 != 0u && (need & ~tp1) == 0u) return 1;
+  return -1;
+}
+
+template <int KH, int KW, int BN, int WM, int WN, unsigned TP0, unsigned TP1, int KGS>
+int launch_group(GroupArgs& g, const oflow_conv_problem* pr, int count, hipStream_t s) {
+  for (int i = 0; i < 2; ++i)
+    g.var[i] = live_variant(pr[i < count ? i : 0].step_live, g.p[i].kg, KH * KW, TP0, TP1, KGS);
+  const ConvArgs& a = g.p[0];
+  const int ntiles = a.tiles_x * a.tiles_y * a.B;
+  const int nblk = g.split + (count > 1 ? g.p[1].npad / BN : 0);
+  hipLaunchKernelGGL((conv_s32_kernel<KH, KW, BN, WM, WN, 0, kTY, kInS32, false, 2, TP0, TP1, KGS, GroupArgs>),
+                     dim3(ntiles, nblk), dim3(64 * WM * WN), 0, s, g.p[0], g);
+  return launch_status();
+}
+
+}
+}
+
+extern "C" int oflow_conv_s32_group(const oflow_conv_problem* problems, int count, int kh, int kw, int block_n,
+                                    void* stream) {
+  if (!problems) return OFLOW_E_NULL;
+  if (count < 1 || count > 2) return OFLOW_E_SHAPE;
+  if (!((kh == 2 && kw == 2 && (block_n == 96 || block_n == 128)) ||
+        (kh == 3 && kw == 3 && (block_n == 64 || block_n == 96))) || OFLOW_XCD_MAP)
+    return OFLOW_E_SHAPE;
+  GroupArgs g{};
+  for (int i = 0; i < count; ++i) {
+    const oflow_conv_problem& p = problems[i];
+    if (i > 0 && (p.B != problems[0].B || p.H != problems[0].H || p.W != problems[0].W)) return OFLOW_E_SHAPE;
+    const int st = build_conv_args(g.p[i], p.d_x, p.x_pixel_stride, p.in_groups, p.d_wpack, p.n_pad, p.d_wscale, p.d_bias,
+                                   p.N, p.B, p.H, p.W, kh, kw, block_n, 0, p.activation, p.out_scale, p.d_y0,
+                                   p.y0_pixel_stride, nullptr, 0, nullptr, 0, 0, 0, nullptr, nullptr, 0, p.d_nhwc,
+                                   p.nhwc_pixel_stride, p.d_stats, nullptr, 0, 0, 0);
+    if (st != OFLOW_OK) return st;
+    if (p.x_pixel_stride & 127) return OFLOW_E_ALIGN;
+    g.p[i].ain = kInS32;
+  }
+  if (count == 1) g.p[1] = g.p[0];
+  g.split = g.p[0].npad / block_n;
+  hipStream_t s = static_cast<hipStream_t>(stream);
+  if (kh == 2) {
+    if (block_n == 96) return launch_group<2, 2, 96, 4, 1, kTapsS2D3x3, kTapsS2D1x1, 8>(g, problems, count, s);
+    return launch_group<2, 2, 128, 2, 2, kTapsS2D3x3, kTapsS2D1x1, 12>(g, problems, count, s);
+  }
+  if (block_n == 96) return launch_group<3, 3, 96, 4, 1, 0u, 0u, 0>(g, problems, count, s);
+  return launch_group<3, 3, 64, 2, 2, 0u, 0u, 0>(g, problems, count, s);
+}
+
 extern "C" int oflow_conv_s32_ex3(const void* d_x, long long x_pixel_stride, int in_groups, const void* d_wpack,
                                   int n_pad, const float* d_wscale, const float* d_bias, int N, int B, int H, int W, int kh,
                                   int kw, int block_n, int epilogue, int activation, float out_scale, void* d_y0,
diff --git a/torch-optical-flow_amd/methods/raft/model/extractor.py b/torch-optical-flow_amd/methods/raft/model/extractor.py
--- a/torch-optical-flow_amd/methods/raft/model/extractor.py
+++ b/torch-optical-flow_amd/methods/raft/model/extractor.py
@@ -10,7 +10,7 @@
 
 from optical_flow import _native
 
-from .update import CONV_BLOCKS, parse_block_overrides
+from .update import CONV_BLOCKS, _env_choice, parse_block_overrides
 
 
 def _norm_layer(norm_fn: str, planes: int, groups: int) -> nn.Module:
@@ -110,6 +110,13 @@
     return out.reshape(n, 4 * c, 2, 2)
 
 
+def _s2d_shortcut_weight(w: Tensor) -> Tensor:
+    n, c = w.shape[:2]
+    out = torch.zeros((n, 4, c, 2, 2), device=w.device, dtype=w.dtype)
+    out[:, 0, :, 1, 1] = w[:, :, 0, 0]
+    return out.reshape(n, 4 * c, 2, 2)
+
+
 def _fold_bn(conv: nn.Conv2d, bn: nn.Module):
     w = conv.weight.detach().double()
     b = conv.bias.detach().double() if conv.bias is not None else torch.zeros(w.shape[0], device=w.device, dtype=w.dtype)
@@ -120,6 +127,10 @@
 
 _ENC_BN_OVERRIDE = {int(k): v for k, v in
                     parse_block_overrides("OFLOW_ENC_BN", {str(b) for b in CONV_BLOCKS}).items()}
+
+
+S2D_TAPSKIP = _env_choice("OFLOW_S2D_TAPSKIP", "1", ("0", "1")) == "1"
+S2D_SHORTCUT_GROUP = _env_choice("OFLOW_S2D_SHORTCUT_GROUP", "0", ("0", "1")) == "1"
 
 
 class SplitEncoder:
@@ -141,10 +152,16 @@
             w, b = conv.weight, conv.bias
         else:
             w, b = _fold_bn(conv, norm)
-        if kw.pop("s2d", False):
+        s2d = kw.pop("s2d", False)
+        if s2d == "shortcut":
+            w = _s2d_shortcut_weight(w.detach().float())
+        elif s2d:
             w = _s2d_weight(w.detach().float())
         n = w.shape[0]
-        return _native.ConvWeights(w, b, ((n + 31) // 32) * 32, **kw)
+        cw = _native.ConvWeights(w, b, ((n + 31) // 32) * 32, **kw)
+        if s2d == "shortcut":
+            cw.cin //= 16
+        return cw
 
     def _pack(self, enc: BasicEncoder):
         W = {"stem": self._cw(enc.conv1, enc.norm1, patches=True)}
@@ -155,6 +172,7 @@
                 W[f"{li}.{bi}.conv2"] = self._cw(blk.conv2, blk.norm2)
                 if s2:
                     W[f"{li}.{bi}.down"] = self._cw(blk.downsample[0], blk.downsample[1])
+                    W[f"{li}.{bi}.down_s2d"] = self._cw(blk.downsample[0], blk.downsample[1], s2d="shortcut")
         W["head"] = _native.ConvWeights(enc.conv2.weight, enc.conv2.bias, ((enc.conv2.out_channels + 31) // 32) * 32)
         return W
 
@@ -201,6 +219,37 @@
             return _native.NhwcNormIn(raw, *shape, alpha, beta)
         return _native.S32Slice(self._conv_norm(x, cw, shape, "relu"))
 
+    def _stride2_head(self, cur, pre: str, shape):
+        b, h, w = shape
+        V, P = _native.S32Slice, _native.ConvProblem
+        cw1, cwd = self.w[pre + "conv1"], self.w[pre + "down"]
+        bn = self._bn(cw1.n)
+        grouped = S2D_SHORTCUT_GROUP and bn in _native.GROUP_SHAPES[(2, 2)] and cw1.n == cwd.n
+        masked1 = (S2D_TAPSKIP or grouped) and bn in _native.GROUP_SHAPES[(2, 2)]
+        if not masked1:
+            t = self._conv1(V(cur), cw1, shape)
+            d = self._conv_norm(V(cur, 0, cwd.kg), cwd, shape, "none", raw_only=True)
+            return t, (d if self.inorm else V(d))
+        dev = cur.device
+        cws = [cw1] + ([self.w[pre + "down_s2d"]] if grouped else [])
+        if self.inorm:
+            tiles = _native.conv_tiles(h, w)
+            raws = [torch.empty((b * h * w, cw.n), device=dev, dtype=torch.float32) for cw in cws]
+            parts = [torch.empty((b, tiles, cw.n_pad, 3), device=dev, dtype=torch.float32) for cw in cws]
+            _native.conv_s32_group([P(V(cur), cw, nhwc=r, stats=q, masked=S2D_TAPSKIP or i > 0)
+                                    for i, (cw, r, q) in enumerate(zip(cws, raws, parts))], bn)
+            norms = [_native.norm_stats(q, b, tiles, cw.n_pad, cw.n, 1e-5) for cw, q in zip(cws, parts)]
+            t = _native.NhwcNormIn(raws[0], b, h, w, *norms[0])
+            if grouped:
+                return t, (raws[1], *norms[1])
+            return t, self._conv_norm(V(cur, 0, cwd.kg), cwd, shape, "none", raw_only=True)
+        outs = [_native.s32_empty(b, h, w, (cw.n + 31) // 32, dev) for cw in cws]
+        _native.conv_s32_group([P(V(cur), cw, act="relu" if i == 0 else "none", y0=V(o), masked=S2D_TAPSKIP or i > 0)
+                                for i, (cw, o) in enumerate(zip(cws, outs))], bn)
+        if grouped:
+            return V(outs[0]), V(outs[1])
+        return V(outs[0]), V(self._conv_norm(V(cur, 0, cwd.kg), cwd, shape, "none", raw_only=True))
+
     def stem_patches(self, x: Tensor) -> Tensor:
         x = x.float().contiguous()
         n, _, hh, ww = x.shape
@@ -252,10 +301,7 @@
                     cur = self._conv_norm(t, self.w[pre + "conv2"], (n, h, w), "relu", res=x_in, s2d=out_s2d)
                 else:
                     h, w = h // 2, w // 2
-                    t = self._conv1(V(cur), self.w[pre + "conv1"], (n, h, w))
-                    cin = self.w[pre + "down"].kg
-                    d = self._conv_norm(V(cur, 0, cin), self.w[pre + "down"], (n, h, w), "none", raw_only=True)
-                    res = d if self.inorm else V(d)
+                    t, res = self._stride2_head(cur, pre, (n, h, w))
                     cur = self._conv_norm(t, self.w[pre + "conv2"], (n, h, w), "relu", res=res, s2d=out_s2d)
                 if out_s2d:
                     pass
diff --git a/torch-optical-flow_amd/methods/raft/model/update.py b/torch-optical-flow_amd/methods/raft/model/update.py
--- a/torch-optical-flow_amd/methods/raft/model/update.py
+++ b/torch-optical-flow_amd/methods/raft/model/update.py
@@ -17,6 +17,8 @@
 CONV_BN = {"c2": 96, "f1": 128, "f2": 64, "mo": 128, "gru": 128, "fh1": 64}
 CONV_BN_SIDE = dict(CONV_BN, c2=64, fh1=128)
 CONV_BLOCKS = (32, 64, 96, 128)
+MOTION_GROUP_BN = 96
+MOTION_GROUP_MIN_PIXELS = 16384
 
 
 def parse_block_overrides(var: str, keys) -> dict:
@@ -44,6 +46,9 @@
 
 for _bn in (CONV_BN, CONV_BN_SIDE):
     _bn.update(parse_block_overrides("OFLOW_CONV_BN", set(CONV_BN)))
+MOTION_GROUP = _env_choice("OFLOW_MOTION_GROUP", "0", ("0", "1")) == "1"
+if os.environ.get("OFLOW_MOTION_GROUP_BN"):
+    MOTION_GROUP_BN = int(_env_choice("OFLOW_MOTION_GROUP_BN", "96", ("64", "96")))
 FLOW_HEAD_MODE = _env_choice("OFLOW_FLOW_HEAD_MODE", "fused", ("fused", "tiled", "conv", "col2im"))
 CONVF1_FROM_FLOW_MIN_PIXELS = 16384 if _env_choice("OFLOW_CONVF1_FROM_FLOW", "1", ("0", "1")) == "1" else 1 << 62
 KSPLIT_LAYERS = frozenset()
@@ -317,6 +322,7 @@
             "c2": CW(enc.convc2.weight, enc.convc2.bias, 192),
             "f1": CW(enc.convf1.weight, enc.convf1.bias, 128, patches=True),
             "f2": CW(enc.convf2.weight, enc.convf2.bias, 64),
+            "f2p96": CW(enc.convf2.weight, enc.convf2.bias, 96),
             "mo": CW(enc.conv.weight, enc.conv.bias, 128),
             "fh1": CW(fh.conv1.weight, fh.conv1.bias, 256),
             "fh2": CW(fh.conv2.weight, fh.conv2.bias, 32),
@@ -385,6 +391,15 @@
             self._convc1(corr_in)
             conv(V(self.c1), w["c2"], bns["c2"], "relu", y0=V(self.cf, 0, 6))
             main.wait_stream(side)
+        elif MOTION_GROUP and b * h * wd >= MOTION_GROUP_MIN_PIXELS:
+            if prep:
+                _native.flow_prep(coords1, self.pm, (V(self.hx), 254), (V(self.rhx), 254))
+            conv(f1_in, w["f1"], bns["f1"], "relu", y0=V(self.f1))
+            self._convc1(corr_in)
+            P = _native.ConvProblem
+            _native.conv_s32_group([P(V(self.c1), w["c2"], act="relu", y0=V(self.cf, 0, 6), masked=False),
+                                    P(V(self.f1), w["f2p96" if MOTION_GROUP_BN == 96 else "f2"], act="relu",
+                                      y0=V(self.cf, 6, 2), masked=False)], MOTION_GROUP_BN)
         else:
             if prep:
                 _native.flow_prep(coords1, self.pm, (V(self.hx), 254), (V(self.rhx), 254))
diff --git a/torch-optical-flow_amd/optical_flow/_native.py b/torch-optical-flow_amd/optical_flow/_native.py
--- a/torch-optical-flow_amd/optical_flow/_native.py
+++ b/torch-optical-flow_amd/optical_flow/_native.py
@@ -68,6 +68,7 @@
     "oflow_range_flag_exchange",
     "oflow_flow_head_col2im_f32",
     "oflow_conv_s32_ex6",
+    "oflow_conv_s32_group",
     "oflow_flow_head_finish_f32",
     "oflow_timing_event_create",
     "oflow_timing_event_destroy",
@@ -77,6 +78,20 @@
     "oflow_sequence_loss_f32",
     "oflow_sequence_loss_backward_f32",
 )
+
+
+
+class ConvProblemC(ctypes.Structure):
+
+    _fields_ = [
+        ("d_x", ctypes.c_void_p), ("x_pixel_stride", ctypes.c_longlong), ("in_groups", ctypes.c_int),
+        ("d_wpack", ctypes.c_void_p), ("n_pad", ctypes.c_int), ("d_wscale", ctypes.c_void_p),
+        ("d_bias", ctypes.c_void_p), ("N", ctypes.c_int), ("B", ctypes.c_int), ("H", ctypes.c_int), ("W", ctypes.c_int),
+        ("step_live", ctypes.c_char_p), ("activation", ctypes.c_int), ("out_scale", ctypes.c_float),
+        ("d_y0", ctypes.c_void_p), ("y0_pixel_stride", ctypes.c_longlong), ("d_nhwc", ctypes.c_void_p),
+        ("nhwc_pixel_stride", ctypes.c_int), ("d_stats", ctypes.c_void_p),
+    ]
+
 
 _lib = None
 _recorder = None
@@ -265,6 +280,8 @@
     lib.oflow_flow_head_col2im_f32.argtypes = [P, P, I, I, I, P, P]
     lib.oflow_conv_s32_ex6.restype = I
     lib.oflow_conv_s32_ex6.argtypes = list(lib.oflow_conv_s32_ex5.argtypes[:-1]) + [P, P, I, P]
+    lib.oflow_conv_s32_group.restype = I
+    lib.oflow_conv_s32_group.argtypes = [ctypes.POINTER(ConvProblemC), I, I, I, I, P]
     lib.oflow_flow_head_finish_f32.restype = I
     lib.oflow_flow_head_finish_f32.argtypes = [P, I, P, I, I, I, P, P, L, P, L, P]
     FP = ctypes.POINTER(F)
@@ -841,7 +858,7 @@
 
 class ConvWeights:
 
-    __slots__ = ("pack", "wscale", "bias", "n", "n_pad", "kh", "kw", "kg", "layout", "cin", "_frag")
+    __slots__ = ("pack", "wscale", "bias", "n", "n_pad", "kh", "kw", "kg", "layout", "cin", "_frag", "live")
 
     def __init__(self, weight: torch.Tensor, bias, n_pad: int, patches: bool = False):
         w = weight.detach().float()
@@ -863,6 +880,7 @@
         hi = full.half()
         lo = (full - hi.float()).half()
         self.pack = torch.stack([hi, lo], dim=3).contiguous()
+        self.live = self.live_steps(self.pack)
         inv = torch.ones(n_pad, device=w.device, dtype=torch.float32)
         inv[:n] = 1.0 / scale
         self.wscale = inv
@@ -873,6 +891,12 @@
         self._frag = None
         if t > 1 and n_pad % 32 == 0:
             self.frag()
+
+    @staticmethod
+    def live_steps(pack: torch.Tensor) -> bytes:
+        kg, t = pack.shape[:2]
+        bits = pack.contiguous().view(torch.int16) & 0x7FFF
+        return bytes((bits != 0).reshape(kg, t, -1).any(dim=2).to(torch.uint8).cpu().reshape(-1).tolist())
 
     def frag(self) -> torch.Tensor:
         if self._frag is None:
@@ -1020,6 +1044,69 @@
         )
 
 
+GROUP_SHAPES = {(2, 2): (96, 128), (3, 3): (64, 96)}
+
+
+class ConvProblem:
+
+    __slots__ = ("x", "cw", "act", "out_scale", "y0", "nhwc", "stats", "masked")
+
+    def __init__(self, x: "S32Slice", cw: "ConvWeights", act: str = "none", out_scale: float = 1.0, y0=None, nhwc=None,
+                 stats=None, masked: bool = True):
+        self.x, self.cw, self.act, self.out_scale = x, cw, act, out_scale
+        self.y0, self.nhwc, self.stats, self.masked = y0, nhwc, stats, masked
+
+
+def conv_s32_group(problems: Sequence["ConvProblem"], block_n: int) -> None:
+    what = "conv_s32_group"
+    if not 1 <= len(problems) <= 2:
+        raise RuntimeError(f"{what}: one or two problems")
+    cw0 = problems[0].cw
+    b, h, w = problems[0].x.bhw
+    dev = problems[0].x.device
+    arr = (ConvProblemC * len(problems))()
+    exec_f16 = useful = 0
+    for i, p in enumerate(problems):
+        cw, x = p.cw, p.x
+        if not isinstance(x, S32Slice) or cw.layout != "conv" or (cw.kh, cw.kw) != (cw0.kh, cw0.kw):
+            raise RuntimeError(f"{what}: S32 inputs and conv-layout weights of one kernel size")
+        if x.ng != cw.kg:
+            raise RuntimeError(f"{what}: input has {x.ng} groups, weights expect {cw.kg}")
+        if x.device != dev:
+            raise RuntimeError(f"{what}: problems on different devices")
+        if CHECK_RANGE:
+            _range_check(x, f"{what} {cw.kh}x{cw.kw}")
+        pb, ph, pw = x.bhw
+        if p.y0 is not None and (tuple(p.y0.t.shape[:3]) != (pb, ph, pw) or p.y0.t.device != dev):
+            raise RuntimeError(f"{what}: destination shape/device mismatch")
+        if p.nhwc is not None and (p.nhwc.dtype != torch.float32 or not p.nhwc.is_contiguous()
+                                   or p.nhwc.numel() != pb * ph * pw * cw.n):
+            raise RuntimeError(f"{what}: nhwc destination must be contiguous fp32 [P, {cw.n}]")
+        if p.stats is not None and (p.stats.dtype != torch.float32 or p.stats.numel() < pb * conv_tiles(ph, pw) * cw.n_pad * 3):
+            raise RuntimeError(f"{what}: stats partials buffer too small")
+        c = arr[i]
+        c.d_x, c.x_pixel_stride, c.in_groups = x.ptr, x.ps, cw.kg
+        c.d_wpack, c.n_pad, c.d_wscale = cw.pack.data_ptr(), cw.n_pad, cw.wscale.data_ptr()
+        c.d_bias = cw.bias.data_ptr() if cw.bias is not None else None
+        c.N, c.B, c.H, c.W = cw.n, pb, ph, pw
+        c.step_live = cw.live if p.masked else None
+        c.activation, c.out_scale = ACT[p.act], float(p.out_scale)
+        c.d_y0 = p.y0.ptr if p.y0 is not None else None
+        c.y0_pixel_stride = p.y0.ps if p.y0 is not None else 0
+        c.d_nhwc = p.nhwc.data_ptr() if p.nhwc is not None else None
+        c.nhwc_pixel_stride = cw.n
+        c.d_stats = p.stats.data_ptr() if p.stats is not None else None
+        taps = cw.kh * cw.kw
+        steps = sum(1 for v in cw.live if v) if p.masked else cw.kg * taps
+        n_exec = -(-cw.n_pad // int(block_n)) * int(block_n)
+        exec_f16 += 3 * 2 * pb * ph * pw * n_exec * 32 * steps
+        useful += 2 * pb * ph * pw * cw.n * cw.cin * taps
+    if _flops is not None:
+        _count(exec_f16, useful)
+    with torch.cuda.device(dev), _Timed(f"conv{cw0.kh}x{cw0.kw}", dev):
+        _check(load().oflow_conv_s32_group(arr, len(problems), cw0.kh, cw0.kw, int(block_n), _stream(dev)), what)
+
+
 def flow_head2(x: "S32Slice", weight: torch.Tensor, bias: torch.Tensor, coords: torch.Tensor) -> None:
     what = "flow_head2"
     b, h, w = x.bhw
```

Result: no change. 469.4 image-pairs/s, median of 6 (+0.7%).
